# hhcho/sfgwas

Measured on AMD Instinct MI355X. Metric: pca_power_iter_ring_macs_per_s, higher is better.
Workload: dtype u64 ring words, exact integers: int8 digits on the matrix core for the MAC of all five moduli, fp64-held integers in the encode and key-switch kernels

## Files before the change

sfgwas_amd/csrc/fp64mod.hpp:

```cpp
#pragma once

#if defined(__HIPCC__) || defined(__CUDACC__)
#define SFG_HD __host__ __device__ __forceinline__
#else
#define SFG_HD inline
#endif

SFG_HD double mulmod_lazy(double x, double w, double wq, double q) {
    double qh = __builtin_rint(x * wq);
    double h = x * w;
    double l = __builtin_fma(x, w, -h);
    double r = __builtin_fma(-qh, q, h);
    return r + l;
}
SFG_HD double mulmod_lazy_q(double x, double w, double q, double qinv) {
    double h = x * w;
    double qh = __builtin_rint(h * qinv);
    double l = __builtin_fma(x, w, -h);
    double r = __builtin_fma(-qh, q, h);
    return r + l;
}
SFG_HD double canon(double x, double q, double qinv) {
    const double r = __builtin_fma(-__builtin_floor(x * qinv), q, x);
    return r == q ? 0.0 : r;
}
SFG_HD double canon_le(double x, double q, double qinv) {
    return __builtin_fma(-__builtin_floor(x * qinv), q, x);
}
SFG_HD double pred(double x, double q, double qinv) {
    double qh = __builtin_rint(x * qinv);
    return __builtin_fma(-qh, q, x);
}

SFG_HD void fwd_stage1_pair(double v0, double v1, double W, double Wq, double q, double qinv, double &r0, double &r1) {
    const double p = mulmod_lazy(v1, W, Wq, q);
    r0 = canon(v0 + p, q, qinv); r1 = canon(v0 - p, q, qinv);
}
```

sfgwas_amd/csrc/kernels.hpp:

```cpp
#pragma once
#include "common.hpp"
#include "mm_plan.hpp"
#include "assoc_plan.hpp"

constexpr int SFG_MAXPATTERN = 128;
struct ModPattern { int period; int8_t m[SFG_MAXPATTERN]; };
struct RowMap { int rpg; size_t gstride_in, gstride_out; };
struct PanelMap { int G, g, shift0; unsigned packed_mask = 0; int K = 0; };

int launch_ntt_fwd(sfg_ctx *ctx, const u64 *in, u64 *out, size_t nrows, const ModPattern &pat);
int launch_ntt_inv(sfg_ctx *ctx, const u64 *in, u64 *out, size_t nrows, const ModPattern &pat);
int launch_ntt_plain(sfg_ctx *ctx, const double *pc, u64 *out, size_t nplain, int L);
struct MoveJob;
struct PtRide;
int launch_ntt_plain_half(sfg_ctx *ctx, const double *pc, u64 *out_half, size_t nplain, int L, PanelMap pm, const uint32_t *perm = nullptr, const MoveJob *mv = nullptr);
int launch_expand_half(sfg_ctx *ctx, const u64 *half, u64 *full, size_t nrows);
int launch_ntt_fwd_map(sfg_ctx *ctx, const u64 *in, u64 *out, size_t nrows, const ModPattern &pat, const RowMap &rm);
int launch_ntt_inv_map(sfg_ctx *ctx, const u64 *in, u64 *out, size_t nrows, const ModPattern &pat, const RowMap &rm);
int launch_ntt_fwd_staged(sfg_ctx *ctx, const u64 *in, u64 *out, size_t nrows, const ModPattern &pat, bool staged);
struct MacStrides { size_t rot_k, rot_r, pt_k, pt_n, out_n, out_r; bool pt_half = false; bool pt_packed = false; bool pt_digits = false; bool i8 = false; bool i8_big = false; bool pt_digits_big = false;
                    const int8_t *B_small = nullptr, *B_big = nullptr;
                    int pt_layout = 0, pt_L = 0;
                    int B_mode = 0;
                    const int8_t *A_small = nullptr, *A_big = nullptr; };
int launch_mac_i8_small(sfg_ctx *ctx, const double *rotf, size_t rotf_k_stride, size_t rotf_r_stride, int plane0, const u64 *pt, u64 *out, int K, int R, int r0, int Ncols,
                        int l0, int nl, int accumulate, const MacStrides &st);
int launch_mac_i8_big(sfg_ctx *ctx, const double *rotf, size_t rotf_k_stride, size_t rotf_r_stride, int plane0, const u64 *pt, u64 *out, int K, int R, int r0, int Ncols,
                      int l0, int accumulate, const MacStrides &st);
int launch_skew(sfg_ctx *ctx, const int8_t *blk, size_t ld, int r, int c, int transposed, int square, int8_t *D);
struct PcCache { double *slot = nullptr; int mode = 0; const uint32_t *perm = nullptr; };
int launch_encode_rows(sfg_ctx *ctx, const int8_t *D, int shift0, int nshift, int L, u64 *pt, bool half_rows = false, int G = 0, int g = 0, unsigned packed_mask = 0, const PcCache *pcache = nullptr,
                       PtRide *ride = nullptr);
int encode_rows_launches(const sfg_ctx *ctx, int nshift);
int i8_ride_prepare(sfg_ctx *ctx, const u64 *panel, int K, int Ncols, size_t pt_k, size_t pt_n, int layout, int L, int launches, PtRide &ride);
int i8_ride_finish(sfg_ctx *ctx, PtRide &ride);
int i8_ride_tiles(sfg_ctx *ctx, int K, int L, int8_t **Bs, int8_t **Bb);
struct I8Args;
void launch_i8_pack_pt_digits(hipStream_t q, const I8Args &a, unsigned items, bool big);
void launch_move_alone(hipStream_t q, const MoveJob &j);
int launch_share(sfg_ctx *ctx, const u64 *rows, size_t rows_ct_stride, const u64 *xr, size_t x_ct_stride, u64 *h, int nl, int nct);
int launch_add_rows(sfg_ctx *ctx, const u64 *a, size_t a_ct_stride, const u64 *b, size_t b_ct_stride, u64 *out, size_t out_ct_stride, int nl, int nct);
int encrypt_errors_moddown(sfg_ctx *ctx, const int32_t *e0, const int32_t *e1, int nct, int level, u64 *out);
int launch_geno_unpack(sfg_ctx *ctx, const sfg_geno *g, size_t r0, size_t c0, size_t nr, size_t nc, int8_t *out, size_t ld_out);
int launch_rotate_right(sfg_ctx *ctx, const u64 *in, u64 *out, int nct, int level, const int *nrot_host);
int launch_rotate_right_indexed(sfg_ctx *ctx, const u64 *in, int nin, u64 *out, int nct, int level, const int *nrot_host, const int *in_index);
int launch_rotate_right_indexed_f64(sfg_ctx *ctx, const u64 *in, int nin, double *outf, int nct, int level, const int *nrot_host, const int *in_index, int L,
                                    const size_t *out_slot = nullptr);
int launch_rotate_right_sum(sfg_ctx *ctx, const u64 *in, int nin, int nct, int level, const int *nrot_host, const int *in_index, const int *group, int nout,
                            u64 *out, size_t out_stride, int accumulate);
int launch_relinearize(sfg_ctx *ctx, const u64 *tmp, int nct, int level, const u64 *mid, u64 *out);
int launch_ct_add(sfg_ctx *ctx, const u64 *a, const u64 *b, u64 *out, size_t nct, int level);
int mac_dma_planes(sfg_ctx *ctx, int L, std::vector<int> &plane_of, std::vector<int> &is_big);
double mac_big_maxterm(u64 q);
int launch_rot_to_f64(sfg_ctx *ctx, const u64 *rot, size_t nrows, int nl_rot, int L, double *rotf);
int launch_mac_dma(sfg_ctx *ctx, const double *rotf, size_t rows_per_k, const u64 *pt, u64 *out, int K, int R, int Ncols, int L, int accumulate, const MacStrides &st,
                   const double *rotsum = nullptr);
int launch_rot_sum(sfg_ctx *ctx, const double *rotf, size_t rows_per_k, int K, int L, double *rotsum);
int launch_pack_pt(sfg_ctx *ctx, const u64 *in, u64 *out, size_t nrows, size_t words_per_row, int L, unsigned packed_mask);
unsigned mac_dma_packed_mask(sfg_ctx *ctx, int L);
bool mac_use_dma(const sfg_ctx *ctx);
int launch_mac_bc(sfg_ctx *ctx, const double *rotf, size_t rows_per_k, const u64 *pt, u64 *out, int K, int R, int Ncols, int L, int accumulate, const MacStrides &st,
                  const double *rotsum);
int rotcache_build_rows_tab(sfg_ctx *ctx, const u64 *A, int s, int in_level, int max_level, int nbr, int b0, int b1, const std::vector<std::vector<uint8_t>> *tabs, double *cache);
int assoc_build_rotcache(sfg_ctx *ctx, const u64 *A_dev, int s, int in_level, int max_level, size_t nr, const std::vector<size_t> &widths, double **out);
struct I8RotPre { int G = 0, nbr = 0, s = 0, L = 0; std::vector<int8_t *> As, Ab; };
int i8_rotpre_build(sfg_ctx *ctx, const u64 *A_dev, int s, int in_level, int max_level, int nbr, const std::vector<std::vector<uint8_t>> *tabs, size_t budget_bytes, const char *prefix, I8RotPre &pre);
void i8_rotpre_free(I8RotPre &pre);
struct I8RotPreScope { I8RotPre pre; ~I8RotPreScope() { i8_rotpre_free(pre); } };
int matmul_resident_range_i8pre(sfg_ctx *ctx, const I8RotPre &pre, int s, int max_level, const sfg_geno *g, unsigned flags, int blk0, int blk1, uint64_t *out);
int matmul_accumulate_i8pre(sfg_ctx *ctx, const I8RotPre &pre, int s, int max_level, const sfg_geno *g, unsigned flags, int j0, int j1, int accumulate, uint64_t *acc,
                            size_t acc_col_words = 0);
int launch_i8_pack_rot_to(sfg_ctx *ctx, const double *rotf, size_t rotf_k_stride, size_t rotf_r_stride, int plane0, int K, int R, int l0, int nl, bool big, int8_t *A_out);
struct AssocRot { double *f64 = nullptr; I8RotPre pre; };
int assoc_build_rot(sfg_ctx *ctx, const u64 *A_dev, int s, int in_level, int max_level, size_t nr, const std::vector<size_t> &widths, AssocRot &out);
void assoc_free_rot(AssocRot &r);
struct AssocRotScope { AssocRot r; ~AssocRotScope() { assoc_free_rot(r); } };
int assoc_product(sfg_ctx *ctx, const AssocRot &r, const uint64_t *A_dev, int s, int in_level, int max_level, const sfg_geno *g, unsigned flags, int nct, uint64_t *out);
int assoc_batch_tail(sfg_ctx *ctx, const u64 *tmp, const sfg_geno *g, int s, size_t nct, size_t ctw, uint64_t *out_dev, size_t out_ct_capacity, size_t out_shift,
                     double *sum_host, double *sqsum_host);

int launch_bed_decode(sfg_ctx *ctx, hipStream_t st, const uint8_t *dbed, size_t bps, size_t num_sample, size_t num_snp, const int32_t *rmap, const int32_t *cmap,
                      int8_t *out, size_t ld);
int launch_bed_decode_lut(sfg_ctx *ctx, hipStream_t st, const uint8_t *dbed, size_t bps, size_t num_sample, size_t num_snp, const int32_t *rmap, const int32_t *cmap,
                          int8_t *out, size_t ld, unsigned lut);
int upload_filter_map(sfg_ctx *ctx, const uint8_t *filt, size_t n, DevMem &map, size_t *kept);

int assoc_stream_part(sfg_ctx *ctx, int fmt, const char *path, size_t num_sample, size_t num_snp, const uint8_t *row_filter, const uint8_t *col_filter,
                      size_t batch_snps, const uint64_t *A_dev, int s, int in_level, int max_level, unsigned flags,
                      uint64_t *out_dev, size_t out_ct_capacity, size_t *out_ct, double *sum_host, double *sqsum_host,
                      int part, int nparts, std::vector<std::pair<size_t, size_t>> *ranges);
```

sfgwas_amd/csrc/ntt.hip:

```cpp
#include "common.hpp"
#include "kernels.hpp"
#include "i8_move.hpp"
#include "ntt_core.hpp"

template <int IN_MODE>
__global__ void __launch_bounds__(512) k_ntt_fwd(const void *in_, u64 *out_, ModPattern pat, RowMap rm, const double *tw_all, const double2 *pack_all, const ModConst *modc) {
    extern __shared__ double lds[];
    const int N = SFG_N, tid = threadIdx.x;
    const size_t row = blockIdx.x;
    const int m = pat.m[row % pat.period];
    const size_t grp = row / rm.rpg, gi = row % rm.rpg;
    if (m == -2) return;
    if (m < 0) {
        const u64 *src = (const u64 *)in_ + grp * rm.gstride_in + gi * N; u64 *dst = out_ + grp * rm.gstride_out + gi * N;
        if (IN_MODE == 0 && src != dst) for (int a = 0; a < 32; a++) dst[a * 512 + tid] = src[a * 512 + tid];
        return;
    }
    const double *tw = tw_all + (size_t)m * N;
    const double2 *pack = pack_all + (size_t)m * (N / 2);
    const double q = modc[m].q, qinv = modc[m].qinv;
    double v[32];
    if (IN_MODE == 0) {
        const u64 *in = (const u64 *)in_ + grp * rm.gstride_in + gi * N;
#pragma unroll
        for (int a = 0; a < 32; a++) v[a] = u64_to_f64(in[a * 512 + tid]);
    } else {
        const double *pc = (const double *)in_ + (row / pat.period) * (size_t)(N / 2);
#pragma unroll
        for (int a = 0; a < 16; a++) v[a] = pred(pc[a * 512 + tid], q, qinv);
#pragma unroll
        for (int a = 16; a < 32; a++) {
            int x = (a - 16) * 512 + tid;
            v[a] = x == 0 ? 0.0 : -pred(pc[N / 2 - x], q, qinv);
        }
    }
    ntt_fwd_phases(v, lds, tw, pack, q, qinv, tid);
    u64 *out = out_ + grp * rm.gstride_out + gi * N;
    {
        const int b = tid >> 4, c = tid & 15;
#pragma unroll
        for (int a = 0; a < 32; a++) out[a * 512 + tid] = f64_to_u64(canon(lds[a * LDS_ROW + c * 33 + b], q, qinv));
    }
}

__global__ void __launch_bounds__(512) k_ntt_inv(const u64 *in_, u64 *out_, ModPattern pat, RowMap rm, const double *tw_all, const double2 *pack_all, const ModConst *modc) {
    extern __shared__ double lds[];
    const int N = SFG_N, tid = threadIdx.x;
    const size_t row = blockIdx.x;
    const int m = pat.m[row % pat.period];
    if (m < 0) return;
    const size_t grp = row / rm.rpg, gi = row % rm.rpg;
    const double *tw = tw_all + (size_t)m * N;
    const double2 *pack = pack_all + (size_t)m * (N / 2);
    const double q = modc[m].q, qinv = modc[m].qinv;
    const u64 *in = in_ + grp * rm.gstride_in + gi * N;
    double v[32];
    {
        const int b = tid >> 4, c = tid & 15;
#pragma unroll
        for (int a = 0; a < 32; a++) lds[a * LDS_ROW + c * 33 + b] = u64_to_f64(in[a * 512 + tid]);
    }
    __syncthreads();
#pragma unroll
    for (int h = 0; h < 2; h++) {
        const int p = tid + 512 * h, a = p >> 5, b = p & 31;
        double w[16];
#pragma unroll
        for (int c = 0; c < 16; c++) w[c] = lds[a * LDS_ROW + c * 33 + b];
        double tl[16];
        {
            const double2 *pk = pack + (size_t)(p >> 6) * 512 + (p & 63);
#pragma unroll
            for (int i = 0; i < 8; i++) { const double2 e = pk[i * 64]; tl[2 * i] = e.x; tl[2 * i + 1] = e.y; }
        }
        gs_stage<16, 1>(w, q, qinv, [&](int g) { return tl[7 + g]; });
        gs_stage<16, 2>(w, q, qinv, [&](int g) { return tl[3 + g]; });
        gs_stage<16, 4>(w, q, qinv, [&](int g) { return tl[1 + g]; });
        gs_stage<16, 8>(w, q, qinv, [&](int g) { return tl[0 + g]; });
#pragma unroll
        for (int c = 0; c < 16; c++) v[h * 16 + c] = pred(w[c], q, qinv);
    }
    __syncthreads();
#pragma unroll
    for (int h = 0; h < 2; h++) {
        const int p = tid + 512 * h, a = p >> 5, b = p & 31;
#pragma unroll
        for (int c = 0; c < 16; c++) lds[a * LDS_ROW + c * 33 + b] = v[h * 16 + c];
    }
    __syncthreads();
    {
        const int a = tid >> 4, c = tid & 15;
#pragma unroll
        for (int b = 0; b < 32; b++) v[b] = lds[a * LDS_ROW + c * 33 + b];
        gs_stage<32, 1>(v, q, qinv, [&](int g) { return tw[512 + a * 16 + g]; });
        gs_stage<32, 2>(v, q, qinv, [&](int g) { return tw[256 + a * 8 + g]; });
        gs_stage<32, 4>(v, q, qinv, [&](int g) { return tw[128 + a * 4 + g]; });
        gs_stage<32, 8>(v, q, qinv, [&](int g) { return tw[64 + a * 2 + g]; });
        gs_stage<32, 16>(v, q, qinv, [&](int g) { return tw[32 + a + g]; });
        __syncthreads();
#pragma unroll
        for (int b = 0; b < 32; b++) lds[a * LDS_ROW + b * 16 + c] = pred(v[b], q, qinv);
    }
    __syncthreads();
#pragma unroll
    for (int a = 0; a < 32; a++) v[a] = lds[a * LDS_ROW + tid];
    gs_stage<32, 1>(v, q, qinv, [&](int g) { return tw[16 + g]; });
    gs_stage<32, 2>(v, q, qinv, [&](int g) { return tw[8 + g]; });
    gs_stage<32, 4>(v, q, qinv, [&](int g) { return tw[4 + g]; });
    gs_stage<32, 8>(v, q, qinv, [&](int g) { return tw[2 + g]; });
    gs_stage<32, 16>(v, q, qinv, [&](int g) { return tw[1 + g]; });
    const double ninv = modc[m].ninv, ninv_q = modc[m].ninv_q;
    u64 *out = out_ + grp * rm.gstride_out + gi * N;
#pragma unroll
    for (int a = 0; a < 32; a++) {
        double x = mulmod_lazy(pred(v[a], q, qinv), ninv, ninv_q, q);
        out[a * 512 + tid] = f64_to_u64(canon(x, q, qinv));
    }
}

constexpr int H3_ROWA = 264;
constexpr int H3_WREG = 4 * 272;
constexpr int H3_DOUBLES = 16 * H3_ROWA > 4 * H3_WREG ? 16 * H3_ROWA : 4 * H3_WREG;
constexpr int H3_LDS_BYTES = H3_DOUBLES * 8;
struct NoFill {};
template <class First, class Store, class Fill = NoFill, bool WIDE = false>
__device__ __forceinline__ void ntt_half3_body(int hs, First first, Store store, double *lds, const double *tw, const double2 *pack, double q, double qinv, int tid, Fill fill = Fill()) {
    double v[32];
    const int a_b = tid >> 4, c_b = tid & 15;
    double w2[2][16];
    if constexpr (std::is_same<Fill, NoFill>::value) {
#pragma unroll
        for (int h = 0; h < 2; h++)
#pragma unroll
            for (int a = 0; a < 16; a++) w2[h][a] = first(a * 512 + tid + 256 * h);
    } else fill(w2);
#pragma unroll
    for (int h = 0; h < 2; h++) {
        double (&w)[16] = w2[h];
        ct_stage<16, 8>(w, q, qinv, [&](int g) { return tw[2 + hs + g]; });
        ct_stage<16, 4>(w, q, qinv, [&](int g) { return tw[4 + 2 * hs + g]; });
        ct_stage<16, 2>(w, q, qinv, [&](int g) { return tw[8 + 4 * hs + g]; });
        ct_stage<16, 1>(w, q, qinv, [&](int g) { return tw[16 + 8 * hs + g]; });
        if (h) __syncthreads();
#pragma unroll
        for (int a = 0; a < 16; a++) lds[a * H3_ROWA + tid] = w[a];
        __syncthreads();
#pragma unroll
        for (int b = 0; b < 16; b++) v[h * 16 + b] = lds[a_b * H3_ROWA + b * 16 + c_b];
    }
    const int ab = 16 * hs + a_b;
    ct_stage<32, 16>(v, q, qinv, [&](int g) { return tw[32 + ab + g]; });
    ct_stage<32, 8>(v, q, qinv, [&](int g) { return tw[64 + ab * 2 + g]; });
    ct_stage<32, 4>(v, q, qinv, [&](int g) { return tw[128 + ab * 4 + g]; });
    ct_stage<32, 2>(v, q, qinv, [&](int g) { return tw[256 + ab * 8 + g]; });
    ct_stage<32, 1>(v, q, qinv, [&](int g) { return tw[512 + ab * 16 + g]; });
    __syncthreads();
    {
        const int wv = tid >> 6, lane = tid & 63, al = lane >> 4, bk = lane & 15;
        double *img = lds + wv * H3_WREG;
        auto sw = [](int idx) { return (idx >> 8) * 272 + ((idx >> 4) & 15) * 17 + (idx & 15); };
#pragma unroll
        for (int r = 0; r < 2; r++) {
            double wc[16];
            __builtin_amdgcn_fence(__ATOMIC_ACQ_REL, "wavefront");
#pragma unroll
            for (int k = 0; k < 16; k++) img[sw(al * 256 + c_b * 16 + k)] = v[16 * r + k];
            __builtin_amdgcn_fence(__ATOMIC_ACQ_REL, "wavefront");
#pragma unroll
            for (int c = 0; c < 16; c++) wc[c] = img[sw(al * 256 + c * 16 + bk)];
            const int p = a_b * 32 + 16 * r + bk;
            double tl[16];
            {
                const double2 *pk = pack + (size_t)((p >> 6) + 8 * hs) * 512 + (p & 63);
#pragma unroll
                for (int i = 0; i < 8; i++) {
                    const double2 e = pk[i * 64];
                    tl[2 * i] = e.x; tl[2 * i + 1] = e.y;
                }
            }
            ct_stage<16, 8>(wc, q, qinv, [&](int g) { return tl[0 + g]; });
            ct_stage<16, 4>(wc, q, qinv, [&](int g) { return tl[1 + g]; });
            ct_stage<16, 2>(wc, q, qinv, [&](int g) { return tl[3 + g]; });
            ct_stage<16, 1>(wc, q, qinv, [&](int g) { return tl[7 + g]; });
            __builtin_amdgcn_fence(__ATOMIC_ACQ_REL, "wavefront");
#pragma unroll
            for (int c = 0; c < 16; c++) img[sw(al * 256 + c * 16 + bk)] = wc[c];
            __builtin_amdgcn_fence(__ATOMIC_ACQ_REL, "wavefront");
#pragma unroll
            for (int ai = 0; ai < 4; ai++) {
                if constexpr (WIDE) {
                    const int x0 = 4 * lane;
                    const int base = ai * 256 + (lane >> 2);
                    store((4 * wv + ai) * 512 + 256 * r + x0, img[sw(base + (4 * (lane & 3) + 0) * 16)], img[sw(base + (4 * (lane & 3) + 1) * 16)],
                          img[sw(base + (4 * (lane & 3) + 2) * 16)], img[sw(base + (4 * (lane & 3) + 3) * 16)]);
                } else {
#pragma unroll
                    for (int qd = 0; qd < 4; qd++) {
                        const int x = qd * 64 + lane;
                        store((4 * wv + ai) * 512 + 256 * r + x, img[sw(ai * 256 + (x & 15) * 16 + (x >> 4))]);
                    }
                }
            }
        }
    }
}
#define NT_ST(p, v) __builtin_nontemporal_store((unsigned)(v), (p))
template <bool PERM, bool DIG>
__device__ __forceinline__ void ntt_half3_wg(size_t vb, double *lds, const double *pc_all, u64 *out_, size_t nplain, int L, PanelMap pm, const double *tw_all, const double2 *pack_all,
                                             const ModConst *modc, const uint32_t *perm) {
    const int N = SFG_N, n = N / 2, tid = threadIdx.x;
    size_t row; int m;
    if (!plain_block_of(vb, nplain, L, row, m)) return;
    const double *tw = tw_all + (size_t)m * N;
    const double2 *pack = pack_all + (size_t)m * (N / 2);
    const double q = modc[m].q, qinv = modc[m].qinv;
    const double *pc = pc_all + (row / L) * (size_t)n;
    unsigned gal = 1;
    if (PERM) { const uint32_t e = perm[pm.shift0 + (int)(row / L)]; pc = pc_all + (size_t)(e & 0xFFFFu) * n; gal = e >> 16; }
    const double W = tw[1], Wq = W * qinv;
    auto first = [&](int j) { const double lo = pc[j], hi = j == 0 ? 0.0 : pc[n - j]; return lo - mulmod_lazy(hi, W, Wq, q); };
    auto fill = [&](double (&w2)[2][16]) {
        double rA[16], rB[16];
#pragma unroll
        for (int k = 0; k < 16; k++) {
            const int i = tid + 256 * k;
            const double lo = pc[i], hi = i == 0 ? 0.0 : pc[n - i];
            const unsigned qd = (((unsigned)i * gal) & (2u * N - 1u)) >> 13;
            const double ca = (qd == 1u || qd == 2u) ? -lo : lo, cb = qd >= 2u ? -hi : hi;
            rA[k] = ca - mulmod_lazy(cb, W, Wq, q);
            rB[k] = cb - mulmod_lazy(ca, W, Wq, q);
        }
#pragma unroll
        for (int h = 0; h < 2; h++) {
#pragma unroll
            for (int k = 0; k < 16; k++) {
                const unsigned raw = ((unsigned)(tid + 256 * k) * gal) & (2u * N - 1u), qd = raw >> 13;
                const int J = qd == 0u ? (int)raw : qd == 1u ? N - (int)raw : qd == 2u ? (int)raw - N : 2 * N - (int)raw, Jb = n - J;
                if (((J >> 8) & 1) == h && J < n) lds[(J >> 9) * H3_ROWA + (J & 255)] = rA[k];
                if (((Jb >> 8) & 1) == h && Jb < n) lds[(Jb >> 9) * H3_ROWA + (Jb & 255)] = rB[k];
            }
            __syncthreads();
#pragma unroll
            for (int a = 0; a < 16; a++) w2[h][a] = lds[a * H3_ROWA + tid];
            __syncthreads();
        }
        if (tid == 0) {
            const double mid = pc[n / 2];
            const double c = ((((unsigned)(n / 2) * gal) & (2u * N - 1u)) >> 13) >= 2u ? -mid : mid;
            w2[0][8] = c - mulmod_lazy(c, W, Wq, q);
        }
    };
    const size_t plain = row / L; const int shift = pm.shift0 + (int)plain;
    const size_t dst = pm.G ? ((size_t)(shift / SFG_D) * pm.G + pm.g) * SFG_D + (size_t)(shift % SFG_D) : plain;
    u64 *out = out_ + (dst * L + m) * (size_t)n;
    size_t dstride = n, cbm = 0;
    if constexpr (DIG) if (pm.packed_mask & PT_COMPACT) {
        const unsigned lm = (1u << L) - 1u, small = pm.packed_mask & lm;
        const int ns_all = __popc(small), ns_below = __popc(small & ((1u << m) - 1u));
        const size_t planes_all = (size_t)ns_all * 5 + (size_t)(L - ns_all) * 6, planes_below = (size_t)ns_below * 5 + (size_t)(m - ns_below) * 6;
        if (pm.packed_mask & PT_KMAJOR) {
            const size_t K = (size_t)pm.K, col = pm.G ? (size_t)(shift / SFG_D) : plain / K, row = pm.G ? (size_t)pm.g * SFG_D + (size_t)(shift % SFG_D) : plain % K;
            out = reinterpret_cast<u64 *>(reinterpret_cast<uint8_t *>(out_) + ((col * planes_all + planes_below) * 64 * K + row) * 128);
            dstride = 64 * K * 128; cbm = K * 128 - 128;
        } else out = reinterpret_cast<u64 *>(reinterpret_cast<uint8_t *>(out_) + dst * (planes_all * n) + planes_below * n);
    }
    if constexpr (DIG) if (!((pm.packed_mask >> m) & 1u) && (pm.packed_mask & PT_DIGITS_BIG)) {
        uint8_t *o8 = reinterpret_cast<uint8_t *>(out);
        auto dig6 = [&](double x, unsigned &lo, unsigned &hi) {
            const u64 b = (u64)__double_as_longlong(canon(x, q, qinv) + (4503599627370496.0 + 141289400074368.0));
            lo = (unsigned)b ^ 0x80808080u; hi = (unsigned)(b >> 32) ^ 0x8080u;
        };
        auto st6 = [&](int j0, double x0, double x1, double x2, double x3) {
            unsigned l0, l1, l2, l3, h0, h1, h2, h3;
            dig6(x0, l0, h0); dig6(x1, l1, h1); dig6(x2, l2, h2); dig6(x3, l3, h3);
            unsigned o[4]; bytes_tr4(l0, l1, l2, l3, o);
            uint8_t *ob = o8 + j0 + (size_t)(j0 >> 7) * cbm;
#pragma unroll
            for (int d = 0; d < 4; d++) NT_ST(reinterpret_cast<unsigned *>(ob + d * dstride), o[d]);
            unsigned p[4]; bytes_tr4(h0, h1, h2, h3, p);
            NT_ST(reinterpret_cast<unsigned *>(ob + 4 * dstride), p[0]);
            NT_ST(reinterpret_cast<unsigned *>(ob + 5 * dstride), p[1]);
        };
        if constexpr (PERM) ntt_half3_body<decltype(first), decltype(st6), decltype(fill), true>(0, first, st6, lds, tw, pack, q, qinv, tid, fill);
        else ntt_half3_body<decltype(first), decltype(st6), NoFill, true>(0, first, st6, lds, tw, pack, q, qinv, tid);
        return;
    }
    if constexpr (DIG) if ((pm.packed_mask >> m) & 1u) {
        uint8_t *o8 = reinterpret_cast<uint8_t *>(out);
        auto dig = [&](double x, unsigned &lo, unsigned &hi) {
            const u64 b = (u64)__double_as_longlong(canon_le(x, q, qinv) + (4503599627370496.0 + 551911719040.0));
            lo = (unsigned)b ^ 0x80808080u; hi = (unsigned)(b >> 32) ^ 0x80u;
        };
        auto st8 = [&](int j0, double x0, double x1, double x2, double x3) {
            unsigned l0, l1, l2, l3, h0, h1, h2, h3;
            dig(x0, l0, h0); dig(x1, l1, h1); dig(x2, l2, h2); dig(x3, l3, h3);
            unsigned o[4]; bytes_tr4(l0, l1, l2, l3, o);
            uint8_t *ob = o8 + j0 + (size_t)(j0 >> 7) * cbm;
#pragma unroll
            for (int d = 0; d < 4; d++) NT_ST(reinterpret_cast<unsigned *>(ob + d * dstride), o[d]);
            NT_ST(reinterpret_cast<unsigned *>(ob + 4 * dstride), (h0 & 255u) | ((h1 & 255u) << 8) | ((h2 & 255u) << 16) | (h3 << 24));
        };
        if constexpr (PERM) ntt_half3_body<decltype(first), decltype(st8), decltype(fill), true>(0, first, st8, lds, tw, pack, q, qinv, tid, fill);
        else ntt_half3_body<decltype(first), decltype(st8), NoFill, true>(0, first, st8, lds, tw, pack, q, qinv, tid);
        return;
    }
    if constexpr (PERM) {
        if (!DIG && ((pm.packed_mask >> m) & 1u)) ntt_half3_body(0, first, [&](int j, double x) { out[j] = pack_limbs_f64(canon_le(x, q, qinv)); }, lds, tw, pack, q, qinv, tid, fill);
        else ntt_half3_body(0, first, [&](int j, double x) { out[j] = f64_to_u64(canon(x, q, qinv)); }, lds, tw, pack, q, qinv, tid, fill);
    } else {
        (void)fill;
        if (!DIG && ((pm.packed_mask >> m) & 1u)) ntt_half3_body(0, first, [&](int j, double x) { out[j] = pack_limbs_f64(canon_le(x, q, qinv)); }, lds, tw, pack, q, qinv, tid);
        else ntt_half3_body(0, first, [&](int j, double x) { out[j] = f64_to_u64(canon(x, q, qinv)); }, lds, tw, pack, q, qinv, tid);
    }
}
template <bool PERM, bool DIG>
__global__ void __launch_bounds__(256, 4) k_ntt_half3(const double *pc_all, u64 *out_, size_t nplain, int L, PanelMap pm, const double *tw_all, const double2 *pack_all, const ModConst *modc,
                                                      const uint32_t *perm) {
    extern __shared__ double lds[];
    ntt_half3_wg<PERM, DIG>(blockIdx.x, lds, pc_all, out_, nplain, L, pm, tw_all, pack_all, modc, perm);
}
template <bool PERM, int DEPTH, bool NT>
__global__ void __launch_bounds__(256, 4) k_ntt_half3_move(const double *pc_all, u64 *out_, size_t nplain, int L, PanelMap pm, const double *tw_all, const double2 *pack_all, const ModConst *modc,
                                                           const uint32_t *perm, MoveJob job) {
    extern __shared__ double lds[];
    if (blockIdx.x < job.nblocks) { i8_move_block<DEPTH, NT>(job, blockIdx.x, reinterpret_cast<unsigned *>(lds), (int)threadIdx.x); return; }
    ntt_half3_wg<PERM, true>((size_t)blockIdx.x - job.nblocks, lds, pc_all, out_, nplain, L, pm, tw_all, pack_all, modc, perm);
}
template <bool STAGED>
__global__ void __launch_bounds__(256, 4) k_ntt_fwd_split(const u64 *in_, u64 *out_, size_t nrows, ModPattern pat, RowMap rm, const double *tw_all, const double2 *pack_all, const ModConst *modc) {
    extern __shared__ double lds[];
    const int N = SFG_N, n = N / 2, tid = threadIdx.x;
    const size_t b = blockIdx.x, row = (b / 16) * 8 + b % 8; const int hs = (int)((b / 8) & 1);
    if (row >= nrows) return;
    const int m = pat.m[row % pat.period];
    const size_t grp = row / rm.rpg, gi = row % rm.rpg;
    const u64 *in = in_ + grp * rm.gstride_in + gi * N;
    u64 *out = out_ + grp * rm.gstride_out + gi * N + (size_t)hs * n;
    if (m == -2) return;
    if (m < 0) {
        for (int k = 0; k < 32; k++) out[k * 256 + tid] = in[(size_t)hs * n + k * 256 + tid];
        return;
    }
    const double *tw = tw_all + (size_t)m * N;
    const double2 *pack = pack_all + (size_t)m * (N / 2);
    const double q = modc[m].q, qinv = modc[m].qinv;
    const double W = hs ? -tw[1] : tw[1], Wq = W * qinv;
    auto first = [&](int j) { return STAGED ? u64_to_f64(in[(size_t)hs * n + j]) : u64_to_f64(in[j]) + mulmod_lazy(u64_to_f64(in[n + j]), W, Wq, q); };
    ntt_half3_body(hs, first, [&](int j, double x) { out[j] = f64_to_u64(canon(x, q, qinv)); }, lds, tw, pack, q, qinv, tid);
}
__global__ void __launch_bounds__(256) k_expand_half(const u64 *half, u64 *full) {
    const int N = SFG_N, n = N / 2; const size_t row = blockIdx.x / (n / 256);
    const int i = (int)(blockIdx.x % (n / 256)) * 256 + threadIdx.x;
    const u64 v = half[row * n + i];
    full[row * N + i] = v; full[row * N + (N - 1 - i)] = v;
}

int ntt_set_attrs(sfg_ctx *ctx) {
    hipError_t e = hipFuncSetAttribute((const void *)k_ntt_fwd<0>, hipFuncAttributeMaxDynamicSharedMemorySize, LDS_DOUBLES * 8);
    if (e == hipSuccess) e = hipFuncSetAttribute((const void *)k_ntt_fwd<1>, hipFuncAttributeMaxDynamicSharedMemorySize, LDS_DOUBLES * 8);
    if (e == hipSuccess) e = hipFuncSetAttribute((const void *)k_ntt_inv, hipFuncAttributeMaxDynamicSharedMemorySize, LDS_DOUBLES * 8);
    if (e == hipSuccess) e = hipFuncSetAttribute((const void *)k_ntt_half3<false, false>, hipFuncAttributeMaxDynamicSharedMemorySize, H3_LDS_BYTES);
    if (e == hipSuccess) e = hipFuncSetAttribute((const void *)k_ntt_half3<true, false>, hipFuncAttributeMaxDynamicSharedMemorySize, H3_LDS_BYTES);
    if (e == hipSuccess) e = hipFuncSetAttribute((const void *)k_ntt_half3<false, true>, hipFuncAttributeMaxDynamicSharedMemorySize, H3_LDS_BYTES);
    if (e == hipSuccess) e = hipFuncSetAttribute((const void *)k_ntt_half3<true, true>, hipFuncAttributeMaxDynamicSharedMemorySize, H3_LDS_BYTES);
    if (e == hipSuccess) e = hipFuncSetAttribute((const void *)k_ntt_fwd_split<false>, hipFuncAttributeMaxDynamicSharedMemorySize, H3_LDS_BYTES);
    if (e == hipSuccess) e = hipFuncSetAttribute((const void *)k_ntt_fwd_split<true>, hipFuncAttributeMaxDynamicSharedMemorySize, H3_LDS_BYTES);
#define SFG_MV_ATTR(P, D, T) if (e == hipSuccess) e = hipFuncSetAttribute((const void *)k_ntt_half3_move<P, D, T>, hipFuncAttributeMaxDynamicSharedMemorySize, H3_LDS_BYTES)
    SFG_MV_ATTR(false, 1, true); SFG_MV_ATTR(true, 1, true);
#ifdef SFG_AB
    SFG_MV_ATTR(false, 1, false); SFG_MV_ATTR(false, 2, false); SFG_MV_ATTR(false, 2, true); SFG_MV_ATTR(false, 3, false); SFG_MV_ATTR(false, 3, true);
    SFG_MV_ATTR(true, 1, false); SFG_MV_ATTR(true, 2, false); SFG_MV_ATTR(true, 2, true); SFG_MV_ATTR(true, 3, false); SFG_MV_ATTR(true, 3, true);
    if (e == hipSuccess && ab_set_attrs(ctx)) return 1;
#endif
#undef SFG_MV_ATTR
    if (e != hipSuccess) SFG_FAIL(ctx, "cannot raise dynamic LDS limit for the NTT kernels");
    return 0;
}

static RowMap dense_map() { RowMap rm; rm.rpg = 1; rm.gstride_in = SFG_N; rm.gstride_out = SFG_N; return rm; }
int launch_ntt_fwd(sfg_ctx *ctx, const u64 *in, u64 *out, size_t nrows, const ModPattern &pat) { return launch_ntt_fwd_map(ctx, in, out, nrows, pat, dense_map()); }
int launch_ntt_inv(sfg_ctx *ctx, const u64 *in, u64 *out, size_t nrows, const ModPattern &pat) { return launch_ntt_inv_map(ctx, in, out, nrows, pat, dense_map()); }
int launch_ntt_fwd_map(sfg_ctx *ctx, const u64 *in, u64 *out, size_t nrows, const ModPattern &pat, const RowMap &rm) {
    if (!nrows) return 0;
    if (in != out && !ctx->cfg.ntt_fwd_full)
        hipLaunchKernelGGL(k_ntt_fwd_split<false>, dim3((unsigned)((nrows + 7) / 8 * 16)), dim3(256), H3_LDS_BYTES, ctx->stream, in, out, nrows, pat, rm, ctx->tw_fwd, ctx->pack_fwd, ctx->modc);
    else
        hipLaunchKernelGGL(k_ntt_fwd<0>, dim3((unsigned)nrows), dim3(512), LDS_DOUBLES * 8, ctx->stream, (const void *)in, out, pat, rm, ctx->tw_fwd, ctx->pack_fwd, ctx->modc);
    SFG_HIP(ctx, hipGetLastError());
    return 0;
}
int launch_ntt_fwd_staged(sfg_ctx *ctx, const u64 *in, u64 *out, size_t nrows, const ModPattern &pat, bool staged) {
    if (!staged) return launch_ntt_fwd(ctx, in, out, nrows, pat);
    if (!nrows) return 0;
    if (in == out) SFG_FAIL(ctx, "forward NTT: rows staged through stage 1 are transformed out of place");
    hipLaunchKernelGGL(k_ntt_fwd_split<true>, dim3((unsigned)((nrows + 7) / 8 * 16)), dim3(256), H3_LDS_BYTES, ctx->stream, in, out, nrows, pat, dense_map(), ctx->tw_fwd, ctx->pack_fwd, ctx->modc);
    SFG_HIP(ctx, hipGetLastError());
    return 0;
}
int launch_ntt_plain(sfg_ctx *ctx, const double *pc, u64 *out, size_t nplain, int L) {
    if (!nplain) return 0;
    ModPattern pat; pat.period = L; for (int l = 0; l < L; l++) pat.m[l] = (int8_t)l;
    hipLaunchKernelGGL(k_ntt_fwd<1>, dim3((unsigned)(nplain * L)), dim3(512), LDS_DOUBLES * 8, ctx->stream, (const void *)pc, out, pat, dense_map(), ctx->tw_fwd, ctx->pack_fwd, ctx->modc);
    SFG_HIP(ctx, hipGetLastError());
    return 0;
}
template <bool PERM>
static int launch_half3_move(sfg_ctx *ctx, dim3 grid, const double *pc, u64 *out_half, size_t nplain, int L, PanelMap pm, const uint32_t *perm, const MoveJob &j) {
#define SFG_MV(D, T) hipLaunchKernelGGL((k_ntt_half3_move<PERM, D, T>), grid, dim3(256), H3_LDS_BYTES, ctx->stream, pc, out_half, nplain, L, pm, ctx->tw_fwd, ctx->pack_fwd, ctx->modc, perm, j)
    if (j.depth == 1 && j.nt) { SFG_MV(1, true); return 0; }
#ifdef SFG_AB
    if (j.depth == 3) { if (j.nt) SFG_MV(3, true); else SFG_MV(3, false); return 0; }
    if (j.depth == 2) { if (j.nt) SFG_MV(2, true); else SFG_MV(2, false); return 0; }
    if (j.depth == 1) { SFG_MV(1, false); return 0; }
#endif
#undef SFG_MV
    SFG_FAIL(ctx, "plaintext NTT: the product build holds the mover with one unit in flight and streaming accesses only (other forms: make ab)");
}
int launch_ntt_plain_half(sfg_ctx *ctx, const double *pc, u64 *out_half, size_t nplain, int L, PanelMap pm, const uint32_t *perm, const MoveJob *mv) {
    if (!nplain) return 0;
    const dim3 grid((unsigned)((nplain + 7) / 8 * 8 * L));
    const bool dig = pm.packed_mask & PT_DIGITS;
    if (mv && mv->count) {
        if (!dig || mv->nblocks % 8 || !mv->nblocks) SFG_FAIL(ctx, "plaintext NTT: mover workgroups need the digit-plane form and a multiple of 8 of them");
        const dim3 g2(grid.x + mv->nblocks);
        if (perm) SFG_TRY(launch_half3_move<true>(ctx, g2, pc, out_half, nplain, L, pm, perm, *mv));
        else SFG_TRY(launch_half3_move<false>(ctx, g2, pc, out_half, nplain, L, pm, (const uint32_t *)nullptr, *mv));
        SFG_HIP(ctx, hipGetLastError());
        return 0;
    }
    if (perm && dig) hipLaunchKernelGGL((k_ntt_half3<true, true>), grid, dim3(256), H3_LDS_BYTES, ctx->stream, pc, out_half, nplain, L, pm, ctx->tw_fwd, ctx->pack_fwd, ctx->modc, perm);
    else if (perm) hipLaunchKernelGGL((k_ntt_half3<true, false>), grid, dim3(256), H3_LDS_BYTES, ctx->stream, pc, out_half, nplain, L, pm, ctx->tw_fwd, ctx->pack_fwd, ctx->modc, perm);
    else if (dig) hipLaunchKernelGGL((k_ntt_half3<false, true>), grid, dim3(256), H3_LDS_BYTES, ctx->stream, pc, out_half, nplain, L, pm, ctx->tw_fwd, ctx->pack_fwd, ctx->modc, (const uint32_t *)nullptr);
#ifdef SFG_AB
    else if (ctx->cfg.ntt_half_full) ab_launch_ntt_half_full(ctx, pc, out_half, nplain, L, pm);
#endif
    else hipLaunchKernelGGL((k_ntt_half3<false, false>), grid, dim3(256), H3_LDS_BYTES, ctx->stream, pc, out_half, nplain, L, pm, ctx->tw_fwd, ctx->pack_fwd, ctx->modc, (const uint32_t *)nullptr);
    SFG_HIP(ctx, hipGetLastError());
    return 0;
}
int launch_expand_half(sfg_ctx *ctx, const u64 *half, u64 *full, size_t nrows) {
    if (!nrows) return 0;
    hipLaunchKernelGGL(k_expand_half, dim3((unsigned)(nrows * (SFG_N / 2 / 256))), dim3(256), 0, ctx->stream, half, full);
    SFG_HIP(ctx, hipGetLastError());
    return 0;
}
int launch_ntt_inv_map(sfg_ctx *ctx, const u64 *in, u64 *out, size_t nrows, const ModPattern &pat, const RowMap &rm) {
    if (!nrows) return 0;
    hipLaunchKernelGGL(k_ntt_inv, dim3((unsigned)nrows), dim3(512), LDS_DOUBLES * 8, ctx->stream, in, out, pat, rm, ctx->tw_inv, ctx->pack_inv, ctx->modc);
    SFG_HIP(ctx, hipGetLastError());
    return 0;
}

static int pattern_from_host(sfg_ctx *ctx, const int *mod_idx, int nrows, ModPattern &pat) {
    for (int period = 1; period <= 64 && period <= nrows; period++) {
        bool ok = true;
        for (int r = 0; r < nrows && ok; r++) ok = mod_idx[r] == mod_idx[r % period];
        if (ok) { pat.period = period; for (int i = 0; i < period; i++) { if (mod_idx[i] < 0 || mod_idx[i] >= ctx->nmod) SFG_FAIL(ctx, "modulus index out of range"); pat.m[i] = (int8_t)mod_idx[i]; } return 0; }
    }
    SFG_FAIL(ctx, "mod_idx must be periodic with period <= 64");
}

extern "C" int sfg_ntt_rows(sfg_ctx *ctx, uint64_t *rows, int nrows, const int *mod_idx) {
    SFG_HIP(ctx, hipSetDevice(ctx->device));
    ModPattern pat; SFG_TRY(pattern_from_host(ctx, mod_idx, nrows, pat));
    return launch_ntt_fwd(ctx, (const u64 *)rows, (u64 *)rows, nrows, pat);
}
extern "C" int sfg_intt_rows(sfg_ctx *ctx, uint64_t *rows, int nrows, const int *mod_idx) {
    SFG_HIP(ctx, hipSetDevice(ctx->device));
    ModPattern pat; SFG_TRY(pattern_from_host(ctx, mod_idx, nrows, pat));
    return launch_ntt_inv(ctx, (const u64 *)rows, (u64 *)rows, nrows, pat);
}
```

sfgwas_amd/csrc/rotate.hip:

```cpp
#include "common.hpp"
#include "kernels.hpp"
#include "ksw.hpp"


static void fill_ext(const sfg_ctx *ctx, ExtConst &e, const std::vector<int> &src) {
    memset(&e, 0, sizeof e);
    e.a = (int)src.size();
    for (int m = 0; m < e.a; m++) e.src[m] = src[m];
    for (int m = 0; m < e.a; m++) {
        u64 qm = ctx->q[src[m]], h = 1;
        for (int k = 0; k < e.a; k++) if (k != m) h = h_mulmod(h, ctx->q[src[k]] % qm, qm);
        u64 hi = h_invmod(h, qm);
        e.qhat_inv[m] = (double)hi; e.qhat_inv_q[m] = (double)hi / (double)qm;
    }
    for (int t = 0; t < ctx->nmod; t++) {
        u64 qt = ctx->q[t], D = 1 % qt;
        for (int m = 0; m < e.a; m++) {
            u64 ht = 1 % qt;
            for (int k = 0; k < e.a; k++) if (k != m) ht = h_mulmod(ht, ctx->q[src[k]] % qt, qt);
            e.qhat_t[t][m] = (double)ht; e.qhat_t_q[t][m] = (double)ht / (double)qt;
            D = h_mulmod(D, ctx->q[src[m]] % qt, qt);
        }
        e.D_t[t] = (double)D; e.D_t_q[t] = (double)D / (double)qt;
    }
}


int get_ksw(sfg_ctx *ctx, int level, KswConst **dev, KswConst *host) {
    KswConst kc; memset(&kc, 0, sizeof kc);
    kc.level = level; kc.nl = level + 1; kc.np = ctx->np; kc.alpha = ctx->np; kc.nt = kc.nl + kc.np;
    kc.beta = (kc.nl + kc.alpha - 1) / kc.alpha;
    if (kc.alpha > KSW_MAXA || kc.beta > KSW_MAXDIG) SFG_FAIL(ctx, "key-switch shape unsupported (alpha > 4 or beta > 8)");
    if (kc.beta * kc.nt > SFG_MAXPATTERN) SFG_FAIL(ctx, "key-switch shape unsupported (beta * (level + 1 + np) = %d rows exceed the modulus pattern table)", kc.beta * kc.nt);
    for (int t = 0; t < kc.nt; t++) { kc.tmod[t] = t < kc.nl ? t : ctx->nq + (t - kc.nl); kc.digit_of[t] = t < kc.nl ? t / kc.alpha : -1; }
    for (int i = 0; i < kc.beta; i++) {
        std::vector<int> src;
        for (int m = i * kc.alpha; m < (i + 1) * kc.alpha && m < kc.nl; m++) src.push_back(m);
        fill_ext(ctx, kc.dig[i], src);
    }
    std::vector<int> ps; for (int p = 0; p < kc.np; p++) ps.push_back(ctx->nq + p);
    fill_ext(ctx, kc.pq, ps);
    for (int t = 0; t < kc.nl; t++) {
        u64 qt = ctx->q[t], P = 1;
        for (int p = 0; p < kc.np; p++) P = h_mulmod(P, ctx->q[ctx->nq + p] % qt, qt);
        u64 pi = h_invmod(P, qt);
        kc.pinv[t] = (double)pi; kc.pinv_q[t] = (double)pi / (double)qt;
    }
    *host = kc;
    auto it = ctx->ksw_cache.find(level);
    if (it == ctx->ksw_cache.end()) {
        KswConst *d = nullptr;
        SFG_HIP(ctx, hipMalloc(&d, sizeof(KswConst)));
        SFG_HIP(ctx, hipMemcpy(d, &kc, sizeof(KswConst), hipMemcpyHostToDevice));
        ctx->ksw_cache[level] = d; *dev = d;
    } else *dev = (KswConst *)it->second;
    return 0;
}


template <bool PRE1>
__global__ void __launch_bounds__(256) k_ksw_extend(const u64 *c2, u64 *ext, const KswConst *kcp, const ModConst *modc, const double *tw_fwd) {
    const KswConst &kc = *kcp;
    const int N = SFG_N, n = N / 2, x = blockIdx.x * 256 + threadIdx.x, i = blockIdx.y; const size_t b = blockIdx.z;
    const ExtConst &e = kc.dig[i];
    const u64 *c2b = c2 + b * (size_t)kc.nl * N;
    u64 *eb = ext + (b * kc.beta + i) * (size_t)kc.nt * N;
    double xs[2][KSW_MAXA], y[2][KSW_MAXA], v[2] = {0.0, 0.0};
#pragma unroll
    for (int h = 0; h < 2; h++)
#pragma unroll
        for (int m = 0; m < KSW_MAXA; m++) xs[h][m] = m < e.a ? u64_to_f64(c2b[(size_t)e.src[m] * N + h * n + x]) : 0.0;
    if (e.a > 1) { ext_prepare(e, modc, xs[0], y[0], v[0]); ext_prepare(e, modc, xs[1], y[1], v[1]); }
    for (int t = 0; t < kc.nt; t++) {
        const int tg = kc.tmod[t];
        if (kc.digit_of[t] == i) continue;
        const double q = modc[tg].q, qinv = modc[tg].qinv;
        double o0, o1;
        if (e.a == 1) { o0 = canon(xs[0][0], q, qinv); o1 = canon(xs[1][0], q, qinv); }
        else { o0 = ext_target(e, tg, q, qinv, y[0], v[0]); o1 = ext_target(e, tg, q, qinv, y[1], v[1]); }
        if (PRE1) { const double W = tw_fwd[(size_t)tg * N + 1]; fwd_stage1_pair(o0, o1, W, W * qinv, q, qinv, o0, o1); }
        eb[(size_t)t * N + x] = f64_to_u64(o0); eb[(size_t)t * N + n + x] = f64_to_u64(o1);
    }
}

__global__ void __launch_bounds__(256) k_ksw_inner(const u64 *ext, const u64 *ct_in, const u64 *const *keys, const int *inidx, u64 *acc, const KswConst *kcp, const ModConst *modc, int nmod, int nq_out) {
    const KswConst &kc = *kcp;
    const int N = SFG_N, x = 2 * (blockIdx.x * 256 + threadIdx.x), t = (int)blockIdx.y < nq_out ? (int)blockIdx.y : (int)blockIdx.y + (kc.nl - nq_out); const size_t b = blockIdx.z;
    const int tg = kc.tmod[t];
    const double q = modc[tg].q, qinv = modc[tg].qinv;
    const u64 *key = keys[b];
    const size_t bi = (size_t)inidx[b];
    double a0x = 0.0, a0y = 0.0, a1x = 0.0, a1y = 0.0;
    for (int i = 0; i < kc.beta; i++) {
        const ulonglong2 ev = kc.digit_of[t] == i ? *reinterpret_cast<const ulonglong2 *>(ct_in + (bi * 2 * (size_t)kc.nl + kc.nl + t) * N + x)
                                                  : *reinterpret_cast<const ulonglong2 *>(ext + ((bi * kc.beta + i) * (size_t)kc.nt + t) * N + x);
        const ulonglong2 k0 = *reinterpret_cast<const ulonglong2 *>(key + (((size_t)i * 2 + 0) * nmod + tg) * N + x);
        const ulonglong2 k1 = *reinterpret_cast<const ulonglong2 *>(key + (((size_t)i * 2 + 1) * nmod + tg) * N + x);
        const double ex = u64_to_f64(ev.x), ey = u64_to_f64(ev.y);
        a0x += mulmod2(ex, u64_to_f64(k0.x), q, qinv); a0y += mulmod2(ey, u64_to_f64(k0.y), q, qinv);
        a1x += mulmod2(ex, u64_to_f64(k1.x), q, qinv); a1y += mulmod2(ey, u64_to_f64(k1.y), q, qinv);
    }
    *reinterpret_cast<ulonglong2 *>(acc + ((b * 2 + 0) * (size_t)kc.nt + t) * N + x) = make_ulonglong2(f64_to_u64(canon(a0x, q, qinv)), f64_to_u64(canon(a0y, q, qinv)));
    *reinterpret_cast<ulonglong2 *>(acc + ((b * 2 + 1) * (size_t)kc.nt + t) * N + x) = make_ulonglong2(f64_to_u64(canon(a1x, q, qinv)), f64_to_u64(canon(a1y, q, qinv)));
}

template <bool PRE1>
__global__ void __launch_bounds__(256) k_moddown_extend(const u64 *acc, u64 *ext2, const KswConst *kcp, const ModConst *modc, const double *tw_fwd, int nq_out) {
    const KswConst &kc = *kcp;
    const int N = SFG_N, n = N / 2, x = blockIdx.x * 256 + threadIdx.x, p = blockIdx.y; const size_t b = blockIdx.z;
    const ExtConst &e = kc.pq;
    const u64 *ap = acc + ((b * 2 + p) * (size_t)kc.nt + kc.nl) * N;
    double xs[2][KSW_MAXA], y[2][KSW_MAXA], v[2] = {0.0, 0.0};
#pragma unroll
    for (int h = 0; h < 2; h++)
#pragma unroll
        for (int m = 0; m < KSW_MAXA; m++) xs[h][m] = m < e.a ? u64_to_f64(ap[(size_t)m * N + h * n + x]) : 0.0;
    if (e.a > 1) { ext_prepare(e, modc, xs[0], y[0], v[0]); ext_prepare(e, modc, xs[1], y[1], v[1]); }
    for (int t = 0; t < nq_out; t++) {
        const double q = modc[t].q, qinv = modc[t].qinv;
        double o0, o1;
        if (e.a == 1) { o0 = canon(xs[0][0], q, qinv); o1 = canon(xs[1][0], q, qinv); }
        else { o0 = ext_target(e, t, q, qinv, y[0], v[0]); o1 = ext_target(e, t, q, qinv, y[1], v[1]); }
        if (PRE1) { const double W = tw_fwd[(size_t)t * N + 1]; fwd_stage1_pair(o0, o1, W, W * qinv, q, qinv, o0, o1); }
        u64 *row = ext2 + ((b * 2 + p) * (size_t)kc.nl + t) * N;
        row[x] = f64_to_u64(o0); row[n + x] = f64_to_u64(o1);
    }
}

struct F64Form { int on, L, centre; size_t rowf; int plane_of[SFG_MAXMOD], big[SFG_MAXMOD]; };
__device__ __forceinline__ void store_rot_f64(double *row, const F64Form &ff, int t, int x, double v, double q) {
    const int N = SFG_N;
    double *o = row + (size_t)ff.plane_of[t] * N;
    if (ff.big[t]) {
        const double wc = v > __builtin_floor(q * 0.5) ? v - q : v;
        const double hi = __builtin_floor((wc + 4194304.0) * 0x1p-23), lo = wc - hi * 8388608.0;
        o[2 * x] = lo; o[2 * x + 1] = hi;
    } else o[x] = (ff.centre && v > __builtin_floor(q * 0.5)) ? v - q : v;
}
__global__ void __launch_bounds__(256) k_ksw_finish(const u64 *ct_in, const int *inidx, const u64 *acc, const u64 *ext2, const uint16_t *const *index,
                                                   u64 *const *ct_out, const KswConst *kcp, const ModConst *modc, const u64 *add1, F64Form ff) {
    const KswConst &kc = *kcp;
    const int N = SFG_N, x = blockIdx.x * 256 + threadIdx.x, t = blockIdx.y; const size_t b = blockIdx.z;
    if (ff.on && t >= ff.L) return;
    const double q = modc[t].q, qinv = modc[t].qinv, pinv = kc.pinv[t], pinv_q = kc.pinv_q[t];
    const int src = index[b][x];
#pragma unroll
    for (int p = 0; p < 2; p++) {
        const double a = u64_to_f64(acc[((b * 2 + p) * (size_t)kc.nt + t) * N + src]);
        const double e = u64_to_f64(ext2[((b * 2 + p) * (size_t)kc.nl + t) * N + src]);
        double r = mulmod_lazy(a - e, pinv, pinv_q, q);
        if (p == 0) r += u64_to_f64(ct_in[((size_t)inidx[b] * 2 * (size_t)kc.nl + t) * N + src]);
        else if (add1) r += u64_to_f64(add1[((size_t)inidx[b] * (size_t)kc.nl + t) * N + src]);
        const double v = canon(r, q, qinv);
        if (ff.on) store_rot_f64(reinterpret_cast<double *>(ct_out[b]) + (size_t)p * ff.rowf, ff, t, x, v, q);
        else ct_out[b][((size_t)p * kc.nl + t) * N + x] = f64_to_u64(v);
    }
}

struct KswSeg { const u64 *plain; u64 *out; int start, count, accumulate, pad; };
__global__ void __launch_bounds__(256) k_ksw_finish_sum(const u64 *ct_in, const int *inidx, const u64 *acc, const u64 *ext2, const uint16_t *const *index,
                                                       const KswSeg *segs, const int *jobs, const KswConst *kcp, const ModConst *modc) {
    const KswConst &kc = *kcp;
    const int N = SFG_N, x = blockIdx.x * 256 + threadIdx.x, t = blockIdx.y;
    const KswSeg sg = segs[blockIdx.z];
    const double q = modc[t].q, qinv = modc[t].qinv, pinv = kc.pinv[t], pinv_q = kc.pinv_q[t];
    const size_t w0 = (size_t)t * N + x, w1 = ((size_t)kc.nl + t) * N + x;
    double s0 = 0.0, s1 = 0.0;
    if (sg.accumulate) { s0 = u64_to_f64(sg.out[w0]); s1 = u64_to_f64(sg.out[w1]); }
    if (sg.plain) { s0 += u64_to_f64(sg.plain[w0]); s1 += u64_to_f64(sg.plain[w1]); }
    for (int k = 0; k < sg.count; k++) {
        const size_t b = (size_t)jobs[sg.start + k];
        const int src = index[b][x];
        const double a0 = u64_to_f64(acc[((b * 2 + 0) * (size_t)kc.nt + t) * N + src]), e0 = u64_to_f64(ext2[((b * 2 + 0) * (size_t)kc.nl + t) * N + src]);
        const double a1 = u64_to_f64(acc[((b * 2 + 1) * (size_t)kc.nt + t) * N + src]), e1 = u64_to_f64(ext2[((b * 2 + 1) * (size_t)kc.nl + t) * N + src]);
        const double c0 = u64_to_f64(ct_in[((size_t)inidx[b] * 2 * (size_t)kc.nl + t) * N + src]);
        s0 += canon(mulmod_lazy(a0 - e0, pinv, pinv_q, q) + c0, q, qinv);
        s1 += canon(mulmod_lazy(a1 - e1, pinv, pinv_q, q), q, qinv);
        if ((k & 7) == 7) { s0 = pred(s0, q, qinv); s1 = pred(s1, q, qinv); }
    }
    sg.out[w0] = f64_to_u64(canon(s0, q, qinv)); sg.out[w1] = f64_to_u64(canon(s1, q, qinv));
}

__global__ void __launch_bounds__(256) k_ct_add(const u64 *a, const u64 *b, u64 *out, int nl, const ModConst *modc, size_t total_rows) {
    const int N = SFG_N; const size_t row = blockIdx.x / (N / 256); const int m = (int)(row % nl);
    const u64 q = modc[m].qi;
    const size_t off = row * N + (blockIdx.x % (N / 256)) * 256 + threadIdx.x;
    u64 v = a[off] + b[off]; out[off] = v >= q ? v - q : v;
}

struct KswSum { int nout; std::vector<int> group; std::vector<const u64 *> plain; u64 *out; size_t out_stride; int accumulate; };
static int launch_keyswitch_jobs(sfg_ctx *ctx, const u64 *in, int nin, int level, const std::vector<int> &job_in, const std::vector<const u64 *> &keyp,
                                 const std::vector<const uint16_t *> &idxp, const std::vector<u64 *> &outp, const u64 *add1, const F64Form *ffp = nullptr,
                                 const KswSum *sum = nullptr) {
    const int N = SFG_N, nl = level + 1;
    F64Form ff; memset(&ff, 0, sizeof ff); if (ffp) ff = *ffp;
    KswConst *kcd; KswConst kc;
    SFG_TRY(get_ksw(ctx, level, &kcd, &kc));
    const size_t ctw = (size_t)2 * nl * N;
    const int nr = (int)job_in.size(), nout = sum ? sum->nout : 0;
    if (sum && (ff.on || add1 || (int)sum->group.size() != nr || (int)sum->plain.size() != nout)) SFG_FAIL(ctx, "key switch: internal: malformed sum groups");
    if (!nr && !nout) return 0;
    const int nq_out = ff.on ? ff.L : nl;
    const bool pre1 = !ctx->cfg.ntt_fwd_full;
    const size_t in_rows = (size_t)nl + (size_t)kc.beta * kc.nt, job_rows = 2 * (size_t)kc.nt + 2 * (size_t)nl;
    const size_t budget = ctx->cfg.ksw_budget;
    int in_grp = (int)(budget / (in_rows * N * 8)); if (in_grp < 1) in_grp = 1; if (in_grp > nin) in_grp = nin;
    int chunk = (int)(budget / (job_rows * N * 8)); if (chunk < 1) chunk = 1; if (chunk > nr) chunk = nr;
    const size_t ptr_bytes = (size_t)nr * (3 * sizeof(void *) + 2 * sizeof(int)) + (size_t)nout * sizeof(KswSeg) + 256;
    const size_t ext_rows = (size_t)in_grp * kc.beta * kc.nt, ext2_rows = (size_t)chunk * 2 * nl;
    SFG_TRY(sfg_ws_reserve(ctx, (in_rows * in_grp + job_rows * chunk + ext_rows + ext2_rows) * N * 8 + ptr_bytes));
    u64 *c2 = (u64 *)ctx->ws, *ext = c2 + (size_t)in_grp * nl * N;
    u64 *acc = ext + ext_rows * N, *ext2 = acc + (size_t)chunk * 2 * kc.nt * N;
    u64 *extT = ext2 + ext2_rows * N, *ext2T = extT + ext_rows * N;
    const u64 **keys_all = (const u64 **)(ext2T + ext2_rows * N);
    const uint16_t **idx_all = (const uint16_t **)(keys_all + nr);
    u64 **out_all = (u64 **)(idx_all + nr);
    KswSeg *segs_d = (KswSeg *)(out_all + nr);
    int *inidx_all = (int *)(segs_d + nout);
    int *segjobs_d = inidx_all + nr;
    std::vector<char> seen(nout, 0);
    std::vector<KswSeg> segs; std::vector<int> segjobs;
    auto finish_sum = [&](const std::vector<int> &jobs, size_t c0, int nb, const u64 *bin, const int *inidx_d, const uint16_t **idx_d) -> int {
        std::vector<int> cnt(nout, 0), at(nout, 0);
        for (int k = 0; k < nb; k++) cnt[sum->group[jobs[c0 + k]]]++;
        segs.clear(); segjobs.assign(nb, 0);
        for (int i = 0, start = 0; i < nout; i++) {
            if (nb ? !cnt[i] : seen[i]) continue;
            KswSeg sg; sg.plain = seen[i] ? nullptr : sum->plain[i]; sg.out = sum->out + (size_t)i * sum->out_stride;
            sg.start = start; sg.count = cnt[i]; sg.accumulate = (sum->accumulate || seen[i]) ? 1 : 0; sg.pad = 0;
            at[i] = start; start += cnt[i]; seen[i] = 1; segs.push_back(sg);
        }
        for (int k = 0; k < nb; k++) segjobs[at[sum->group[jobs[c0 + k]]]++] = k;
        if (segs.empty()) return 0;
        SFG_TRY(sfg_upload_small(ctx, segs_d, segs.data(), segs.size() * sizeof(KswSeg)));
        SFG_TRY(sfg_upload_small(ctx, segjobs_d, segjobs.data(), (size_t)nb * sizeof(int)));
        hipLaunchKernelGGL(k_ksw_finish_sum, dim3(N / 256, nl, (unsigned)segs.size()), dim3(256), 0, ctx->stream, bin, inidx_d, acc, ext2T, idx_d, segs_d, segjobs_d, kcd, ctx->modc);
        SFG_HIP(ctx, hipGetLastError());
        return 0;
    };
    ModPattern pq; pq.period = nl; for (int m = 0; m < nl; m++) pq.m[m] = m < nq_out ? (int8_t)m : (int8_t)-2;
    ModPattern pin; pin.period = nl; for (int m = 0; m < nl; m++) pin.m[m] = (int8_t)m;
    ModPattern pext; pext.period = kc.beta * kc.nt;
    for (int i = 0; i < kc.beta; i++) for (int t = 0; t < kc.nt; t++)
        pext.m[i * kc.nt + t] = (kc.digit_of[t] == i || (t >= nq_out && t < nl)) ? (int8_t)-2 : (int8_t)kc.tmod[t];
    ModPattern pp; pp.period = kc.np; for (int p = 0; p < kc.np; p++) pp.m[p] = (int8_t)(ctx->nq + p);
    for (int i0 = 0; i0 < nin; i0 += in_grp) {
        const int ni = nin - i0 < in_grp ? nin - i0 : in_grp;
        std::vector<int> jobs;
        for (int k = 0; k < nr; k++) if (job_in[k] >= i0 && job_in[k] < i0 + ni) jobs.push_back(k);
        if (jobs.empty()) continue;
        const u64 *bin = in + (size_t)i0 * ctw;
        RowMap rm1; rm1.rpg = nl; rm1.gstride_in = ctw; rm1.gstride_out = (size_t)nl * N;
        SFG_TRY(launch_ntt_inv_map(ctx, bin + (size_t)nl * N, c2, (size_t)ni * nl, pin, rm1));
        if (pre1) hipLaunchKernelGGL(k_ksw_extend<true>, dim3(N / 512, kc.beta, ni), dim3(256), 0, ctx->stream, c2, ext, kcd, ctx->modc, ctx->tw_fwd);
        else hipLaunchKernelGGL(k_ksw_extend<false>, dim3(N / 512, kc.beta, ni), dim3(256), 0, ctx->stream, c2, ext, kcd, ctx->modc, ctx->tw_fwd);
        SFG_HIP(ctx, hipGetLastError());
        SFG_TRY(launch_ntt_fwd_staged(ctx, ext, extT, (size_t)ni * kc.beta * kc.nt, pext, pre1));
        {
            const size_t nj = jobs.size();
            std::vector<const u64 *> kp(nj); std::vector<const uint16_t *> ip(nj); std::vector<u64 *> op(nj); std::vector<int> ii(nj);
            for (size_t k = 0; k < nj; k++) { int jb = jobs[k]; kp[k] = keyp[jb]; ip[k] = idxp[jb]; op[k] = sum ? nullptr : outp[jb]; ii[k] = job_in[jb] - i0; }
            SFG_TRY(sfg_upload_small(ctx, keys_all, kp.data(), nj * sizeof(void *)));
            SFG_TRY(sfg_upload_small(ctx, idx_all, ip.data(), nj * sizeof(void *)));
            if (!sum) SFG_TRY(sfg_upload_small(ctx, out_all, op.data(), nj * sizeof(void *)));
            SFG_TRY(sfg_upload_small(ctx, inidx_all, ii.data(), nj * sizeof(int)));
        }
        for (size_t c0 = 0; c0 < jobs.size(); c0 += chunk) {
            const int nb = (int)(jobs.size() - c0 < (size_t)chunk ? jobs.size() - c0 : (size_t)chunk);
            const u64 **keys_d = keys_all + c0; const uint16_t **idx_d = idx_all + c0; u64 **out_d = out_all + c0; int *inidx_d = inidx_all + c0;
            hipLaunchKernelGGL(k_ksw_inner, dim3(N / 512, nq_out + kc.np, nb), dim3(256), 0, ctx->stream, extT, bin, keys_d, inidx_d, acc, kcd, ctx->modc, ctx->nmod, nq_out);
            SFG_HIP(ctx, hipGetLastError());
            RowMap rm4; rm4.rpg = kc.np; rm4.gstride_in = (size_t)kc.nt * N; rm4.gstride_out = (size_t)kc.nt * N;
            SFG_TRY(launch_ntt_inv_map(ctx, acc + (size_t)nl * N, acc + (size_t)nl * N, (size_t)nb * 2 * kc.np, pp, rm4));
            if (pre1) hipLaunchKernelGGL(k_moddown_extend<true>, dim3(N / 512, 2, nb), dim3(256), 0, ctx->stream, acc, ext2, kcd, ctx->modc, ctx->tw_fwd, nq_out);
            else hipLaunchKernelGGL(k_moddown_extend<false>, dim3(N / 512, 2, nb), dim3(256), 0, ctx->stream, acc, ext2, kcd, ctx->modc, ctx->tw_fwd, nq_out);
            SFG_HIP(ctx, hipGetLastError());
            SFG_TRY(launch_ntt_fwd_staged(ctx, ext2, ext2T, (size_t)nb * 2 * nl, pq, pre1));
            if (sum) { SFG_TRY(finish_sum(jobs, c0, nb, bin, inidx_d, idx_d)); continue; }
            hipLaunchKernelGGL(k_ksw_finish, dim3(N / 256, nq_out, nb), dim3(256), 0, ctx->stream, bin, inidx_d, acc, ext2T, idx_d, out_d, kcd, ctx->modc,
                               add1 ? add1 + (size_t)i0 * nl * N : nullptr, ff);
            SFG_HIP(ctx, hipGetLastError());
        }
    }
    if (sum) SFG_TRY(finish_sum(std::vector<int>(), 0, 0, in, inidx_all, idx_all));
    return 0;
}
int launch_rotate_right_indexed(sfg_ctx *ctx, const u64 *in, int nin, u64 *out, int nct, int level, const int *nrot_host, const int *in_index) {
    const int N = SFG_N, nl = level + 1;
    if (level < 0 || level >= ctx->nq) SFG_FAIL(ctx, "rotate: level out of range");
    const size_t ctw = (size_t)2 * nl * N;
    std::vector<int> job_in; std::vector<const u64 *> keyp; std::vector<const uint16_t *> idxp; std::vector<u64 *> outp;
    for (int j = 0; j < nct; j++) {
        int nrot = nrot_host[j] % SFG_SLOTS; if (nrot < 0) nrot += SFG_SLOTS;
        const int src = in_index ? in_index[j] : j;
        if (src < 0 || src >= nin) SFG_FAIL(ctx, "rotate: input index out of range");
        if (nrot == 0) {
            int run = 1;
            while (j + run < nct && (nrot_host[j + run] % SFG_SLOTS) == 0 && (in_index ? in_index[j + run] : j + run) == src + run && src + run < nin) run++;
            SFG_HIP(ctx, hipMemcpyAsync(out + j * ctw, in + (size_t)src * ctw, (size_t)run * ctw * 8, hipMemcpyDeviceToDevice, ctx->stream));
            j += run - 1;
            continue;
        }
        u64 g = sfg_galois_for_rotation(ctx, SFG_SLOTS - nrot);
        auto it = ctx->rotkeys().find(g);
        if (it == ctx->rotkeys().end()) SFG_FAIL(ctx, "rotate: no rotation key loaded for right-rotation by %d (galois element %llu)", nrot, g);
        job_in.push_back(src); keyp.push_back(it->second.key_dev); idxp.push_back(it->second.index_dev); outp.push_back(out + j * ctw);
    }
    return launch_keyswitch_jobs(ctx, in, nin, level, job_in, keyp, idxp, outp, nullptr);
}
int launch_rotate_right_sum(sfg_ctx *ctx, const u64 *in, int nin, int nct, int level, const int *nrot_host, const int *in_index, const int *group, int nout,
                            u64 *out, size_t out_stride, int accumulate) {
    const int N = SFG_N, nl = level + 1;
    if (level < 0 || level >= ctx->nq) SFG_FAIL(ctx, "rotate: level out of range");
    const size_t ctw = (size_t)2 * nl * N;
    KswSum sum; sum.nout = nout; sum.plain.assign(nout, nullptr); sum.out = out; sum.out_stride = out_stride; sum.accumulate = accumulate;
    std::vector<int> job_in; std::vector<const u64 *> keyp; std::vector<const uint16_t *> idxp;
    for (int j = 0; j < nct; j++) {
        int nrot = nrot_host[j] % SFG_SLOTS; if (nrot < 0) nrot += SFG_SLOTS;
        const int src = in_index ? in_index[j] : j;
        if (src < 0 || src >= nin) SFG_FAIL(ctx, "rotate: input index out of range");
        if (group[j] < 0 || group[j] >= nout) SFG_FAIL(ctx, "rotate: sum group out of range");
        if (nrot == 0) {
            if (sum.plain[group[j]]) SFG_FAIL(ctx, "rotate: more than one unrotated member in a sum group");
            sum.plain[group[j]] = in + (size_t)src * ctw;
            continue;
        }
        u64 g = sfg_galois_for_rotation(ctx, SFG_SLOTS - nrot);
        auto it = ctx->rotkeys().find(g);
        if (it == ctx->rotkeys().end()) SFG_FAIL(ctx, "rotate: no rotation key loaded for right-rotation by %d (galois element %llu)", nrot, g);
        job_in.push_back(src); keyp.push_back(it->second.key_dev); idxp.push_back(it->second.index_dev); sum.group.push_back(group[j]);
    }
    return launch_keyswitch_jobs(ctx, in, nin, level, job_in, keyp, idxp, std::vector<u64 *>(), nullptr, nullptr, &sum);
}
int launch_rotate_right_indexed_f64(sfg_ctx *ctx, const u64 *in, int nin, double *outf, int nct, int level, const int *nrot_host, const int *in_index, int L,
                                    const size_t *out_slot) {
    const int N = SFG_N, nl = level + 1;
    ctx->i8_gen++;
    if (level < 0 || level >= ctx->nq || L > nl) SFG_FAIL(ctx, "rotate: level out of range");
    const size_t ctw = (size_t)2 * nl * N;
    std::vector<int> plane_of, is_big; const int nplanes = mac_dma_planes(ctx, L, plane_of, is_big);
    if (nplanes < 0) return 1;
    F64Form ff; memset(&ff, 0, sizeof ff);
    ff.on = 1; ff.L = L; ff.centre = mac_dma_packed_mask(ctx, L) != 0; ff.rowf = (size_t)nplanes * N;
    for (int l = 0; l < L; l++) { ff.plane_of[l] = plane_of[l]; ff.big[l] = is_big[l]; }
    std::vector<int> job_in; std::vector<const u64 *> keyp; std::vector<const uint16_t *> idxp; std::vector<u64 *> outp;
    for (int j = 0; j < nct; j++) {
        int nrot = nrot_host[j] % SFG_SLOTS; if (nrot < 0) nrot += SFG_SLOTS;
        const int src = in_index ? in_index[j] : j;
        if (src < 0 || src >= nin) SFG_FAIL(ctx, "rotate: input index out of range");
        double *dst = outf + (out_slot ? out_slot[j] : (size_t)j) * 2 * ff.rowf;
        if (nrot == 0) {
            int run = 1;
            while (!out_slot && j + run < nct && (nrot_host[j + run] % SFG_SLOTS) == 0 && (in_index ? in_index[j + run] : j + run) == src + run && src + run < nin) run++;
            SFG_TRY(launch_rot_to_f64(ctx, in + (size_t)src * ctw, (size_t)2 * run, nl, L, dst));
            j += run - 1;
            continue;
        }
        u64 g = sfg_galois_for_rotation(ctx, SFG_SLOTS - nrot);
        auto it = ctx->rotkeys().find(g);
        if (it == ctx->rotkeys().end()) SFG_FAIL(ctx, "rotate: no rotation key loaded for right-rotation by %d (galois element %llu)", nrot, g);
        job_in.push_back(src); keyp.push_back(it->second.key_dev); idxp.push_back(it->second.index_dev); outp.push_back(reinterpret_cast<u64 *>(dst));
    }
    return launch_keyswitch_jobs(ctx, in, nin, level, job_in, keyp, idxp, outp, nullptr, &ff);
}
int launch_relinearize(sfg_ctx *ctx, const u64 *tmp, int nct, int level, const u64 *mid, u64 *out) {
    auto it = ctx->rotkeys().find(1);
    if (it == ctx->rotkeys().end()) SFG_FAIL(ctx, "relinearize: no relinearisation key loaded");
    const size_t ctw = (size_t)2 * (level + 1) * SFG_N;
    std::vector<int> job_in(nct); std::vector<const u64 *> keyp(nct, it->second.key_dev); std::vector<const uint16_t *> idxp(nct, it->second.index_dev); std::vector<u64 *> outp(nct);
    for (int j = 0; j < nct; j++) { job_in[j] = j; outp[j] = out + (size_t)j * ctw; }
    return launch_keyswitch_jobs(ctx, tmp, nct, level, job_in, keyp, idxp, outp, mid);
}
int launch_rotate_right(sfg_ctx *ctx, const u64 *in, u64 *out, int nct, int level, const int *nrot_host) {
    return launch_rotate_right_indexed(ctx, in, nct, out, nct, level, nrot_host, nullptr);
}

extern "C" int sfg_rotate_right_dev(sfg_ctx *ctx, const uint64_t *in, uint64_t *out, int nct, int level, const int *nrot_host) {
    SFG_HIP(ctx, hipSetDevice(ctx->device));
    if (in == out) SFG_FAIL(ctx, "rotate: in and out must not alias");
    PhaseTimer t(ctx, "rotate");
    int rc = launch_rotate_right(ctx, (const u64 *)in, (u64 *)out, nct, level, nrot_host);
    t.stop(1);
    return rc;
}

extern "C" int sfg_ct_galois_dev(sfg_ctx *ctx, const uint64_t *in, uint64_t *out, int nct, int level, uint64_t galois_el) {
    SFG_HIP(ctx, hipSetDevice(ctx->device));
    if (in == out) SFG_FAIL(ctx, "galois: in and out must not alias");
    if (level < 0 || level >= ctx->nq) SFG_FAIL(ctx, "galois: level out of range");
    auto it = ctx->rotkeys().find(galois_el);
    if (it == ctx->rotkeys().end() || galois_el == 1) SFG_FAIL(ctx, "galois: no switching key loaded for galois element %llu", (unsigned long long)galois_el);
    const size_t ctw = (size_t)2 * (level + 1) * SFG_N;
    std::vector<int> job_in(nct); std::vector<const u64 *> keyp(nct, it->second.key_dev); std::vector<const uint16_t *> idxp(nct, it->second.index_dev); std::vector<u64 *> outp(nct);
    for (int j = 0; j < nct; j++) { job_in[j] = j; outp[j] = (u64 *)out + (size_t)j * ctw; }
    PhaseTimer t(ctx, "rotate");
    int rc = launch_keyswitch_jobs(ctx, (const u64 *)in, nct, level, job_in, keyp, idxp, outp, nullptr);
    t.stop(1);
    return rc;
}

int launch_ct_add(sfg_ctx *ctx, const u64 *a, const u64 *b, u64 *out, size_t nct, int level) {
    const int nl = level + 1; const size_t rows = nct * 2 * nl;
    if (!rows) return 0;
    hipLaunchKernelGGL(k_ct_add, dim3((unsigned)(rows * (SFG_N / 256))), dim3(256), 0, ctx->stream, a, b, out, nl, ctx->modc, rows);
    SFG_HIP(ctx, hipGetLastError());
    return 0;
}
extern "C" int sfg_ct_add_dev(sfg_ctx *ctx, const uint64_t *a, const uint64_t *b, uint64_t *out, int nct, int level) {
    SFG_HIP(ctx, hipSetDevice(ctx->device));
    if (level < 0 || level >= ctx->nq) SFG_FAIL(ctx, "evaluator op: level %d out of range", level);
    if (nct < 0) SFG_FAIL(ctx, "evaluator op: negative ciphertext count");
    return launch_ct_add(ctx, (const u64 *)a, (const u64 *)b, (u64 *)out, (size_t)nct, level);
}
```

Baseline: 6342 billion.

## Restructure key-switch: split inverse NTT, tile jobs sharing keys, fuse q-part inner product into finish

Adds a split inverse NTT kernel that leaves the last butterfly stage undone, folding it into the extend and moddown kernels that follow. The key-switch inner product now groups consecutive jobs that share a key and index table into tiles of up to three, so each key load serves several ciphertexts. The inner kernel now covers only the special primes, while the q-modulus inner product is recomputed inside the finish kernels. This is meant to cut key memory traffic, launch work and accumulator size, at the cost of more complex kernels and more register pressure.

After: 6481 billion, median of 6. 1.02x the previous value.

```diff
diff --git a/sfgwas_amd/csrc/fp64mod.hpp b/sfgwas_amd/csrc/fp64mod.hpp
--- a/sfgwas_amd/csrc/fp64mod.hpp
+++ b/sfgwas_amd/csrc/fp64mod.hpp
@@ -36,3 +36,6 @@
     const double p = mulmod_lazy(v1, W, Wq, q);
     r0 = canon(v0 + p, q, qinv); r1 = canon(v0 - p, q, qinv);
 }
+SFG_HD void inv_last_pair(double U, double V, double ninv, double ninv_q, double wn, double wn_q, double q, double qinv, double &r0, double &r1) {
+    r0 = canon(mulmod_lazy(U + V, ninv, ninv_q, q), q, qinv); r1 = canon(mulmod_lazy(U - V, wn, wn_q, q), q, qinv);
+}
diff --git a/sfgwas_amd/csrc/kernels.hpp b/sfgwas_amd/csrc/kernels.hpp
--- a/sfgwas_amd/csrc/kernels.hpp
+++ b/sfgwas_amd/csrc/kernels.hpp
@@ -18,6 +18,7 @@
 int launch_ntt_fwd_map(sfg_ctx *ctx, const u64 *in, u64 *out, size_t nrows, const ModPattern &pat, const RowMap &rm);
 int launch_ntt_inv_map(sfg_ctx *ctx, const u64 *in, u64 *out, size_t nrows, const ModPattern &pat, const RowMap &rm);
 int launch_ntt_fwd_staged(sfg_ctx *ctx, const u64 *in, u64 *out, size_t nrows, const ModPattern &pat, bool staged);
+int launch_ntt_inv_split(sfg_ctx *ctx, const u64 *in, u64 *out, size_t nrows, const ModPattern &pat, const RowMap &rm);
 struct MacStrides { size_t rot_k, rot_r, pt_k, pt_n, out_n, out_r; bool pt_half = false; bool pt_packed = false; bool pt_digits = false; bool i8 = false; bool i8_big = false; bool pt_digits_big = false;
                     const int8_t *B_small = nullptr, *B_big = nullptr;
                     int pt_layout = 0, pt_L = 0;
diff --git a/sfgwas_amd/csrc/ksw_plan.hpp b/sfgwas_amd/csrc/ksw_plan.hpp
--- /dev/null
+++ b/sfgwas_amd/csrc/ksw_plan.hpp
@@ -0,0 +1,30 @@
+#pragma once
+#include <cstddef>
+#include <vector>
+
+struct KswTile { int start, count; };
+
+template <class K, class I>
+inline void ksw_job_tiles(const K *key, const I *tab, int nb, int T, std::vector<KswTile> &tiles) {
+    tiles.clear();
+    if (T < 1) T = 1;
+    for (int k = 0; k < nb;) {
+        int n = 1;
+        while (k + n < nb && n < T && key[k + n] == key[k] && tab[k + n] == tab[k]) n++;
+        tiles.push_back(KswTile{k, n});
+        k += n;
+    }
+}
+
+struct KswSegPlan { int out, start, count, first; };
+inline void ksw_plan_segments(const int *group, int nb, int nout, std::vector<char> &seen, std::vector<KswSegPlan> &segs, std::vector<int> &segjobs) {
+    std::vector<int> cnt((size_t)nout, 0), at((size_t)nout, 0);
+    for (int k = 0; k < nb; k++) cnt[(size_t)group[k]]++;
+    segs.clear(); segjobs.assign((size_t)nb, 0);
+    for (int i = 0, start = 0; i < nout; i++) {
+        if (nb ? !cnt[(size_t)i] : (bool)seen[(size_t)i]) continue;
+        segs.push_back(KswSegPlan{i, start, cnt[(size_t)i], seen[(size_t)i] ? 0 : 1});
+        at[(size_t)i] = start; start += cnt[(size_t)i]; seen[(size_t)i] = 1;
+    }
+    for (int k = 0; k < nb; k++) segjobs[(size_t)at[(size_t)group[k]]++] = k;
+}
diff --git a/sfgwas_amd/csrc/ntt.hip b/sfgwas_amd/csrc/ntt.hip
--- a/sfgwas_amd/csrc/ntt.hip
+++ b/sfgwas_amd/csrc/ntt.hip
@@ -348,6 +348,82 @@
     auto first = [&](int j) { return STAGED ? u64_to_f64(in[(size_t)hs * n + j]) : u64_to_f64(in[j]) + mulmod_lazy(u64_to_f64(in[n + j]), W, Wq, q); };
     ntt_half3_body(hs, first, [&](int j, double x) { out[j] = f64_to_u64(canon(x, q, qinv)); }, lds, tw, pack, q, qinv, tid);
 }
+__global__ void __launch_bounds__(256, 4) k_ntt_inv_split(const u64 *in_, u64 *out_, size_t nrows, ModPattern pat, RowMap rm, const double *tw_all, const double2 *pack_all, const ModConst *modc) {
+    extern __shared__ double lds[];
+    const int N = SFG_N, n = N / 2, tid = threadIdx.x;
+    const size_t blk = blockIdx.x, row = (blk / 16) * 8 + blk % 8; const int hs = (int)((blk / 8) & 1);
+    if (row >= nrows) return;
+    const int m = pat.m[row % pat.period];
+    if (m < 0) return;
+    const size_t grp = row / rm.rpg, gi = row % rm.rpg;
+    const u64 *in = in_ + grp * rm.gstride_in + gi * N + (size_t)hs * n;
+    u64 *out = out_ + grp * rm.gstride_out + gi * N + (size_t)hs * n;
+    const double *tw = tw_all + (size_t)m * N;
+    const double2 *pack = pack_all + (size_t)m * (N / 2);
+    const double q = modc[m].q, qinv = modc[m].qinv;
+    const int a_b = tid >> 4, c_b = tid & 15;
+    double v[32];
+    {
+        const int wv = tid >> 6, lane = tid & 63, al = lane >> 4, bk = lane & 15;
+        double *img = lds + wv * H3_WREG;
+        auto sw = [](int idx) { return (idx >> 8) * 272 + ((idx >> 4) & 15) * 17 + (idx & 15); };
+#pragma unroll
+        for (int r = 0; r < 2; r++) {
+            double wc[16];
+            __builtin_amdgcn_fence(__ATOMIC_ACQ_REL, "wavefront");
+#pragma unroll
+            for (int ai = 0; ai < 4; ai++)
+#pragma unroll
+                for (int qd = 0; qd < 4; qd++) {
+                    const int x = qd * 64 + lane;
+                    img[sw(ai * 256 + (x & 15) * 16 + (x >> 4))] = u64_to_f64(in[(4 * wv + ai) * 512 + 256 * r + x]);
+                }
+            __builtin_amdgcn_fence(__ATOMIC_ACQ_REL, "wavefront");
+#pragma unroll
+            for (int c = 0; c < 16; c++) wc[c] = img[sw(al * 256 + c * 16 + bk)];
+            const int p = a_b * 32 + 16 * r + bk;
+            double tl[16];
+            {
+                const double2 *pk = pack + (size_t)((p >> 6) + 8 * hs) * 512 + (p & 63);
+#pragma unroll
+                for (int i = 0; i < 8; i++) { const double2 e = pk[i * 64]; tl[2 * i] = e.x; tl[2 * i + 1] = e.y; }
+            }
+            gs_stage<16, 1>(wc, q, qinv, [&](int g) { return tl[7 + g]; });
+            gs_stage<16, 2>(wc, q, qinv, [&](int g) { return tl[3 + g]; });
+            gs_stage<16, 4>(wc, q, qinv, [&](int g) { return tl[1 + g]; });
+            gs_stage<16, 8>(wc, q, qinv, [&](int g) { return tl[0 + g]; });
+            __builtin_amdgcn_fence(__ATOMIC_ACQ_REL, "wavefront");
+#pragma unroll
+            for (int c = 0; c < 16; c++) img[sw(al * 256 + c * 16 + bk)] = pred(wc[c], q, qinv);
+            __builtin_amdgcn_fence(__ATOMIC_ACQ_REL, "wavefront");
+#pragma unroll
+            for (int k = 0; k < 16; k++) v[16 * r + k] = img[sw(al * 256 + c_b * 16 + k)];
+        }
+    }
+    const int ab = 16 * hs + a_b;
+    gs_stage<32, 1>(v, q, qinv, [&](int g) { return tw[512 + ab * 16 + g]; });
+    gs_stage<32, 2>(v, q, qinv, [&](int g) { return tw[256 + ab * 8 + g]; });
+    gs_stage<32, 4>(v, q, qinv, [&](int g) { return tw[128 + ab * 4 + g]; });
+    gs_stage<32, 8>(v, q, qinv, [&](int g) { return tw[64 + ab * 2 + g]; });
+    gs_stage<32, 16>(v, q, qinv, [&](int g) { return tw[32 + ab + g]; });
+    __syncthreads();
+#pragma unroll
+    for (int h = 0; h < 2; h++) {
+        double w[16];
+        if (h) __syncthreads();
+#pragma unroll
+        for (int b = 0; b < 16; b++) lds[a_b * H3_ROWA + b * 16 + c_b] = pred(v[h * 16 + b], q, qinv);
+        __syncthreads();
+#pragma unroll
+        for (int a = 0; a < 16; a++) w[a] = lds[a * H3_ROWA + tid];
+        gs_stage<16, 1>(w, q, qinv, [&](int g) { return tw[16 + 8 * hs + g]; });
+        gs_stage<16, 2>(w, q, qinv, [&](int g) { return tw[8 + 4 * hs + g]; });
+        gs_stage<16, 4>(w, q, qinv, [&](int g) { return tw[4 + 2 * hs + g]; });
+        gs_stage<16, 8>(w, q, qinv, [&](int g) { return tw[2 + hs + g]; });
+#pragma unroll
+        for (int a = 0; a < 16; a++) out[a * 512 + tid + 256 * h] = f64_to_u64(canon(w[a], q, qinv));
+    }
+}
 __global__ void __launch_bounds__(256) k_expand_half(const u64 *half, u64 *full) {
     const int N = SFG_N, n = N / 2; const size_t row = blockIdx.x / (n / 256);
     const int i = (int)(blockIdx.x % (n / 256)) * 256 + threadIdx.x;
@@ -365,6 +441,7 @@
     if (e == hipSuccess) e = hipFuncSetAttribute((const void *)k_ntt_half3<true, true>, hipFuncAttributeMaxDynamicSharedMemorySize, H3_LDS_BYTES);
     if (e == hipSuccess) e = hipFuncSetAttribute((const void *)k_ntt_fwd_split<false>, hipFuncAttributeMaxDynamicSharedMemorySize, H3_LDS_BYTES);
     if (e == hipSuccess) e = hipFuncSetAttribute((const void *)k_ntt_fwd_split<true>, hipFuncAttributeMaxDynamicSharedMemorySize, H3_LDS_BYTES);
+    if (e == hipSuccess) e = hipFuncSetAttribute((const void *)k_ntt_inv_split, hipFuncAttributeMaxDynamicSharedMemorySize, H3_LDS_BYTES);
 #define SFG_MV_ATTR(P, D, T) if (e == hipSuccess) e = hipFuncSetAttribute((const void *)k_ntt_half3_move<P, D, T>, hipFuncAttributeMaxDynamicSharedMemorySize, H3_LDS_BYTES)
     SFG_MV_ATTR(false, 1, true); SFG_MV_ATTR(true, 1, true);
 #ifdef SFG_AB
@@ -450,6 +527,12 @@
     SFG_HIP(ctx, hipGetLastError());
     return 0;
 }
+int launch_ntt_inv_split(sfg_ctx *ctx, const u64 *in, u64 *out, size_t nrows, const ModPattern &pat, const RowMap &rm) {
+    if (!nrows) return 0;
+    hipLaunchKernelGGL(k_ntt_inv_split, dim3((unsigned)((nrows + 7) / 8 * 16)), dim3(256), H3_LDS_BYTES, ctx->stream, in, out, nrows, pat, rm, ctx->tw_inv, ctx->pack_inv, ctx->modc);
+    SFG_HIP(ctx, hipGetLastError());
+    return 0;
+}
 
 static int pattern_from_host(sfg_ctx *ctx, const int *mod_idx, int nrows, ModPattern &pat) {
     for (int period = 1; period <= 64 && period <= nrows; period++) {
diff --git a/sfgwas_amd/csrc/rotate.hip b/sfgwas_amd/csrc/rotate.hip
--- a/sfgwas_amd/csrc/rotate.hip
+++ b/sfgwas_amd/csrc/rotate.hip
@@ -1,6 +1,14 @@
 #include "common.hpp"
 #include "kernels.hpp"
 #include "ksw.hpp"
+#include "ksw_plan.hpp"
+
+#ifndef KSW_T
+#define KSW_T 3
+#endif
+#ifndef KSW_INV_SPLIT
+#define KSW_INV_SPLIT true
+#endif
 
 
 static void fill_ext(const sfg_ctx *ctx, ExtConst &e, const std::vector<int> &src) {
@@ -58,8 +66,12 @@
 }
 
 
-template <bool PRE1>
-__global__ void __launch_bounds__(256) k_ksw_extend(const u64 *c2, u64 *ext, const KswConst *kcp, const ModConst *modc, const double *tw_fwd) {
+__device__ __forceinline__ void inv_last_of(const ModConst &mc, double w, double &u, double &v) {
+    const double wn = canon(mulmod_lazy(w, mc.ninv, mc.ninv_q, mc.q), mc.q, mc.qinv);
+    inv_last_pair(u, v, mc.ninv, mc.ninv_q, wn, wn * mc.qinv, mc.q, mc.qinv, u, v);
+}
+template <bool PRE1, bool POST1>
+__global__ void __launch_bounds__(256) k_ksw_extend(const u64 *c2, u64 *ext, const KswConst *kcp, const ModConst *modc, const double *tw_fwd, const double *tw_inv) {
     const KswConst &kc = *kcp;
     const int N = SFG_N, n = N / 2, x = blockIdx.x * 256 + threadIdx.x, i = blockIdx.y; const size_t b = blockIdx.z;
     const ExtConst &e = kc.dig[i];
@@ -70,6 +82,10 @@
     for (int h = 0; h < 2; h++)
 #pragma unroll
         for (int m = 0; m < KSW_MAXA; m++) xs[h][m] = m < e.a ? u64_to_f64(c2b[(size_t)e.src[m] * N + h * n + x]) : 0.0;
+    if (POST1) {
+#pragma unroll
+        for (int m = 0; m < KSW_MAXA; m++) if (m < e.a) inv_last_of(modc[e.src[m]], tw_inv[(size_t)e.src[m] * N + 1], xs[0][m], xs[1][m]);
+    }
     if (e.a > 1) { ext_prepare(e, modc, xs[0], y[0], v[0]); ext_prepare(e, modc, xs[1], y[1], v[1]); }
     for (int t = 0; t < kc.nt; t++) {
         const int tg = kc.tmod[t];
@@ -83,38 +99,58 @@
     }
 }
 
-__global__ void __launch_bounds__(256) k_ksw_inner(const u64 *ext, const u64 *ct_in, const u64 *const *keys, const int *inidx, u64 *acc, const KswConst *kcp, const ModConst *modc, int nmod, int nq_out) {
+template <int T>
+__global__ void __launch_bounds__(256) k_ksw_inner_p(const u64 *ext, const u64 *const *keys, const int *inidx, const KswTile *tiles, u64 *acc, const KswConst *kcp,
+                                                    const ModConst *modc, int nmod) {
     const KswConst &kc = *kcp;
-    const int N = SFG_N, x = 2 * (blockIdx.x * 256 + threadIdx.x), t = (int)blockIdx.y < nq_out ? (int)blockIdx.y : (int)blockIdx.y + (kc.nl - nq_out); const size_t b = blockIdx.z;
+    const int N = SFG_N, x = 2 * (blockIdx.x * 256 + threadIdx.x), m = blockIdx.y, t = kc.nl + m;
+    const KswTile tl = tiles[blockIdx.z];
     const int tg = kc.tmod[t];
     const double q = modc[tg].q, qinv = modc[tg].qinv;
-    const u64 *key = keys[b];
-    const size_t bi = (size_t)inidx[b];
-    double a0x = 0.0, a0y = 0.0, a1x = 0.0, a1y = 0.0;
+    const u64 *key = keys[tl.start];
+    const u64 *eb[T];
+#pragma unroll
+    for (int j = 0; j < T; j++) eb[j] = ext + ((size_t)inidx[tl.start + (j < tl.count ? j : 0)] * kc.beta * (size_t)kc.nt + t) * N + x;
+    double a[T][4];
+#pragma unroll
+    for (int j = 0; j < T; j++) a[j][0] = a[j][1] = a[j][2] = a[j][3] = 0.0;
     for (int i = 0; i < kc.beta; i++) {
-        const ulonglong2 ev = kc.digit_of[t] == i ? *reinterpret_cast<const ulonglong2 *>(ct_in + (bi * 2 * (size_t)kc.nl + kc.nl + t) * N + x)
-                                                  : *reinterpret_cast<const ulonglong2 *>(ext + ((bi * kc.beta + i) * (size_t)kc.nt + t) * N + x);
         const ulonglong2 k0 = *reinterpret_cast<const ulonglong2 *>(key + (((size_t)i * 2 + 0) * nmod + tg) * N + x);
         const ulonglong2 k1 = *reinterpret_cast<const ulonglong2 *>(key + (((size_t)i * 2 + 1) * nmod + tg) * N + x);
-        const double ex = u64_to_f64(ev.x), ey = u64_to_f64(ev.y);
-        a0x += mulmod2(ex, u64_to_f64(k0.x), q, qinv); a0y += mulmod2(ey, u64_to_f64(k0.y), q, qinv);
-        a1x += mulmod2(ex, u64_to_f64(k1.x), q, qinv); a1y += mulmod2(ey, u64_to_f64(k1.y), q, qinv);
-    }
-    *reinterpret_cast<ulonglong2 *>(acc + ((b * 2 + 0) * (size_t)kc.nt + t) * N + x) = make_ulonglong2(f64_to_u64(canon(a0x, q, qinv)), f64_to_u64(canon(a0y, q, qinv)));
-    *reinterpret_cast<ulonglong2 *>(acc + ((b * 2 + 1) * (size_t)kc.nt + t) * N + x) = make_ulonglong2(f64_to_u64(canon(a1x, q, qinv)), f64_to_u64(canon(a1y, q, qinv)));
-}
-
-template <bool PRE1>
-__global__ void __launch_bounds__(256) k_moddown_extend(const u64 *acc, u64 *ext2, const KswConst *kcp, const ModConst *modc, const double *tw_fwd, int nq_out) {
+        const double k0x = u64_to_f64(k0.x), k0y = u64_to_f64(k0.y), k1x = u64_to_f64(k1.x), k1y = u64_to_f64(k1.y);
+#pragma unroll
+        for (int j = 0; j < T; j++) {
+            const ulonglong2 ev = *reinterpret_cast<const ulonglong2 *>(eb[j] + (size_t)i * kc.nt * N);
+            const double ex = u64_to_f64(ev.x), ey = u64_to_f64(ev.y);
+            a[j][0] += mulmod2(ex, k0x, q, qinv); a[j][1] += mulmod2(ey, k0y, q, qinv);
+            a[j][2] += mulmod2(ex, k1x, q, qinv); a[j][3] += mulmod2(ey, k1y, q, qinv);
+        }
+    }
+#pragma unroll
+    for (int j = 0; j < T; j++) {
+        if (j < tl.count) {
+            u64 *o = acc + ((size_t)(tl.start + j) * 2 * kc.np + m) * N + x;
+            *reinterpret_cast<ulonglong2 *>(o) = make_ulonglong2(f64_to_u64(canon(a[j][0], q, qinv)), f64_to_u64(canon(a[j][1], q, qinv)));
+            *reinterpret_cast<ulonglong2 *>(o + (size_t)kc.np * N) = make_ulonglong2(f64_to_u64(canon(a[j][2], q, qinv)), f64_to_u64(canon(a[j][3], q, qinv)));
+        }
+    }
+}
+
+template <bool PRE1, bool POST1>
+__global__ void __launch_bounds__(256) k_moddown_extend(const u64 *acc, u64 *ext2, const KswConst *kcp, const ModConst *modc, const double *tw_fwd, const double *tw_inv, int nq_out) {
     const KswConst &kc = *kcp;
     const int N = SFG_N, n = N / 2, x = blockIdx.x * 256 + threadIdx.x, p = blockIdx.y; const size_t b = blockIdx.z;
     const ExtConst &e = kc.pq;
-    const u64 *ap = acc + ((b * 2 + p) * (size_t)kc.nt + kc.nl) * N;
+    const u64 *ap = acc + (b * 2 + p) * (size_t)kc.np * N;
     double xs[2][KSW_MAXA], y[2][KSW_MAXA], v[2] = {0.0, 0.0};
 #pragma unroll
     for (int h = 0; h < 2; h++)
 #pragma unroll
         for (int m = 0; m < KSW_MAXA; m++) xs[h][m] = m < e.a ? u64_to_f64(ap[(size_t)m * N + h * n + x]) : 0.0;
+    if (POST1) {
+#pragma unroll
+        for (int m = 0; m < KSW_MAXA; m++) if (m < e.a) inv_last_of(modc[e.src[m]], tw_inv[(size_t)e.src[m] * N + 1], xs[0][m], xs[1][m]);
+    }
     if (e.a > 1) { ext_prepare(e, modc, xs[0], y[0], v[0]); ext_prepare(e, modc, xs[1], y[1], v[1]); }
     for (int t = 0; t < nq_out; t++) {
         const double q = modc[t].q, qinv = modc[t].qinv;
@@ -137,29 +173,57 @@
         o[2 * x] = lo; o[2 * x + 1] = hi;
     } else o[x] = (ff.centre && v > __builtin_floor(q * 0.5)) ? v - q : v;
 }
-__global__ void __launch_bounds__(256) k_ksw_finish(const u64 *ct_in, const int *inidx, const u64 *acc, const u64 *ext2, const uint16_t *const *index,
-                                                   u64 *const *ct_out, const KswConst *kcp, const ModConst *modc, const u64 *add1, F64Form ff) {
+template <int T>
+__device__ __forceinline__ void ksw_inner_q(const u64 *ext, const u64 *ct_in, const u64 *key, const KswConst &kc, int nmod, int t, int src, const size_t (&bi)[T],
+                                           double q, double qinv, double (&a)[T][2]) {
+    const int N = SFG_N;
+#pragma unroll
+    for (int j = 0; j < T; j++) a[j][0] = a[j][1] = 0.0;
+    for (int i = 0; i < kc.beta; i++) {
+        const double k0 = u64_to_f64(key[(((size_t)i * 2 + 0) * nmod + t) * N + src]), k1 = u64_to_f64(key[(((size_t)i * 2 + 1) * nmod + t) * N + src]);
+        const bool own = kc.digit_of[t] == i;
+#pragma unroll
+        for (int j = 0; j < T; j++) {
+            const double e = u64_to_f64(own ? ct_in[(bi[j] * 2 * (size_t)kc.nl + kc.nl + t) * N + src] : ext[((bi[j] * kc.beta + i) * (size_t)kc.nt + t) * N + src]);
+            a[j][0] += mulmod2(e, k0, q, qinv); a[j][1] += mulmod2(e, k1, q, qinv);
+        }
+    }
+}
+template <int T>
+__global__ void __launch_bounds__(256) k_ksw_finish(const u64 *ext, const u64 *ct_in, const u64 *const *keys, const int *inidx, const u64 *ext2, const uint16_t *const *index,
+                                                   u64 *const *ct_out, const KswTile *tiles, const KswConst *kcp, const ModConst *modc, int nmod, const u64 *add1, F64Form ff) {
     const KswConst &kc = *kcp;
-    const int N = SFG_N, x = blockIdx.x * 256 + threadIdx.x, t = blockIdx.y; const size_t b = blockIdx.z;
+    const int N = SFG_N, x = blockIdx.x * 256 + threadIdx.x, t = blockIdx.y;
     if (ff.on && t >= ff.L) return;
+    const KswTile tl = tiles[blockIdx.z];
     const double q = modc[t].q, qinv = modc[t].qinv, pinv = kc.pinv[t], pinv_q = kc.pinv_q[t];
-    const int src = index[b][x];
-#pragma unroll
-    for (int p = 0; p < 2; p++) {
-        const double a = u64_to_f64(acc[((b * 2 + p) * (size_t)kc.nt + t) * N + src]);
-        const double e = u64_to_f64(ext2[((b * 2 + p) * (size_t)kc.nl + t) * N + src]);
-        double r = mulmod_lazy(a - e, pinv, pinv_q, q);
-        if (p == 0) r += u64_to_f64(ct_in[((size_t)inidx[b] * 2 * (size_t)kc.nl + t) * N + src]);
-        else if (add1) r += u64_to_f64(add1[((size_t)inidx[b] * (size_t)kc.nl + t) * N + src]);
-        const double v = canon(r, q, qinv);
-        if (ff.on) store_rot_f64(reinterpret_cast<double *>(ct_out[b]) + (size_t)p * ff.rowf, ff, t, x, v, q);
-        else ct_out[b][((size_t)p * kc.nl + t) * N + x] = f64_to_u64(v);
+    const int src = index[tl.start][x];
+    size_t bi[T];
+#pragma unroll
+    for (int j = 0; j < T; j++) bi[j] = (size_t)inidx[tl.start + (j < tl.count ? j : 0)];
+    double a[T][2];
+    ksw_inner_q<T>(ext, ct_in, keys[tl.start], kc, nmod, t, src, bi, q, qinv, a);
+#pragma unroll
+    for (int j = 0; j < T; j++) {
+        if (j < tl.count) {
+            const size_t b = (size_t)(tl.start + j);
+#pragma unroll
+            for (int p = 0; p < 2; p++) {
+                const double e = u64_to_f64(ext2[((b * 2 + p) * (size_t)kc.nl + t) * N + src]);
+                double r = mulmod_lazy(pred(a[j][p], q, qinv) - e, pinv, pinv_q, q);
+                if (p == 0) r += u64_to_f64(ct_in[(bi[j] * 2 * (size_t)kc.nl + t) * N + src]);
+                else if (add1) r += u64_to_f64(add1[(bi[j] * (size_t)kc.nl + t) * N + src]);
+                const double v = canon(r, q, qinv);
+                if (ff.on) store_rot_f64(reinterpret_cast<double *>(ct_out[b]) + (size_t)p * ff.rowf, ff, t, x, v, q);
+                else ct_out[b][((size_t)p * kc.nl + t) * N + x] = f64_to_u64(v);
+            }
+        }
     }
 }
 
 struct KswSeg { const u64 *plain; u64 *out; int start, count, accumulate, pad; };
-__global__ void __launch_bounds__(256) k_ksw_finish_sum(const u64 *ct_in, const int *inidx, const u64 *acc, const u64 *ext2, const uint16_t *const *index,
-                                                       const KswSeg *segs, const int *jobs, const KswConst *kcp, const ModConst *modc) {
+__global__ void __launch_bounds__(256) k_ksw_finish_sum(const u64 *ext, const u64 *ct_in, const u64 *const *keys, const int *inidx, const u64 *ext2, const uint16_t *const *index,
+                                                       const KswSeg *segs, const int *jobs, const KswConst *kcp, const ModConst *modc, int nmod) {
     const KswConst &kc = *kcp;
     const int N = SFG_N, x = blockIdx.x * 256 + threadIdx.x, t = blockIdx.y;
     const KswSeg sg = segs[blockIdx.z];
@@ -170,12 +234,14 @@
     if (sg.plain) { s0 += u64_to_f64(sg.plain[w0]); s1 += u64_to_f64(sg.plain[w1]); }
     for (int k = 0; k < sg.count; k++) {
         const size_t b = (size_t)jobs[sg.start + k];
+        const size_t bi[1] = {(size_t)inidx[b]};
         const int src = index[b][x];
-        const double a0 = u64_to_f64(acc[((b * 2 + 0) * (size_t)kc.nt + t) * N + src]), e0 = u64_to_f64(ext2[((b * 2 + 0) * (size_t)kc.nl + t) * N + src]);
-        const double a1 = u64_to_f64(acc[((b * 2 + 1) * (size_t)kc.nt + t) * N + src]), e1 = u64_to_f64(ext2[((b * 2 + 1) * (size_t)kc.nl + t) * N + src]);
-        const double c0 = u64_to_f64(ct_in[((size_t)inidx[b] * 2 * (size_t)kc.nl + t) * N + src]);
-        s0 += canon(mulmod_lazy(a0 - e0, pinv, pinv_q, q) + c0, q, qinv);
-        s1 += canon(mulmod_lazy(a1 - e1, pinv, pinv_q, q), q, qinv);
+        double a[1][2];
+        ksw_inner_q<1>(ext, ct_in, keys[b], kc, nmod, t, src, bi, q, qinv, a);
+        const double e0 = u64_to_f64(ext2[((b * 2 + 0) * (size_t)kc.nl + t) * N + src]), e1 = u64_to_f64(ext2[((b * 2 + 1) * (size_t)kc.nl + t) * N + src]);
+        const double c0 = u64_to_f64(ct_in[(bi[0] * 2 * (size_t)kc.nl + t) * N + src]);
+        s0 += canon(mulmod_lazy(pred(a[0][0], q, qinv) - e0, pinv, pinv_q, q) + c0, q, qinv);
+        s1 += canon(mulmod_lazy(pred(a[0][1], q, qinv) - e1, pinv, pinv_q, q), q, qinv);
         if ((k & 7) == 7) { s0 = pred(s0, q, qinv); s1 = pred(s1, q, qinv); }
     }
     sg.out[w0] = f64_to_u64(canon(s0, q, qinv)); sg.out[w1] = f64_to_u64(canon(s1, q, qinv));
@@ -206,11 +272,11 @@
     const size_t budget = ctx->cfg.ksw_budget;
     int in_grp = (int)(budget / (in_rows * N * 8)); if (in_grp < 1) in_grp = 1; if (in_grp > nin) in_grp = nin;
     int chunk = (int)(budget / (job_rows * N * 8)); if (chunk < 1) chunk = 1; if (chunk > nr) chunk = nr;
-    const size_t ptr_bytes = (size_t)nr * (3 * sizeof(void *) + 2 * sizeof(int)) + (size_t)nout * sizeof(KswSeg) + 256;
-    const size_t ext_rows = (size_t)in_grp * kc.beta * kc.nt, ext2_rows = (size_t)chunk * 2 * nl;
-    SFG_TRY(sfg_ws_reserve(ctx, (in_rows * in_grp + job_rows * chunk + ext_rows + ext2_rows) * N * 8 + ptr_bytes));
+    const size_t ptr_bytes = (size_t)nr * (3 * sizeof(void *) + 2 * sizeof(int) + sizeof(KswTile)) + (size_t)nout * sizeof(KswSeg) + 256;
+    const size_t ext_rows = (size_t)in_grp * kc.beta * kc.nt, ext2_rows = (size_t)chunk * 2 * nl, acc_rows = (size_t)chunk * 2 * kc.np;
+    SFG_TRY(sfg_ws_reserve(ctx, (in_rows * in_grp + acc_rows + 2 * ext2_rows + ext_rows) * N * 8 + ptr_bytes));
     u64 *c2 = (u64 *)ctx->ws, *ext = c2 + (size_t)in_grp * nl * N;
-    u64 *acc = ext + ext_rows * N, *ext2 = acc + (size_t)chunk * 2 * kc.nt * N;
+    u64 *acc = ext + ext_rows * N, *ext2 = acc + acc_rows * N;
     u64 *extT = ext2 + ext2_rows * N, *ext2T = extT + ext_rows * N;
     const u64 **keys_all = (const u64 **)(ext2T + ext2_rows * N);
     const uint16_t **idx_all = (const uint16_t **)(keys_all + nr);
@@ -218,23 +284,24 @@
     KswSeg *segs_d = (KswSeg *)(out_all + nr);
     int *inidx_all = (int *)(segs_d + nout);
     int *segjobs_d = inidx_all + nr;
+    KswTile *tiles_all = (KswTile *)(segjobs_d + nr);
     std::vector<char> seen(nout, 0);
-    std::vector<KswSeg> segs; std::vector<int> segjobs;
-    auto finish_sum = [&](const std::vector<int> &jobs, size_t c0, int nb, const u64 *bin, const int *inidx_d, const uint16_t **idx_d) -> int {
-        std::vector<int> cnt(nout, 0), at(nout, 0);
-        for (int k = 0; k < nb; k++) cnt[sum->group[jobs[c0 + k]]]++;
-        segs.clear(); segjobs.assign(nb, 0);
-        for (int i = 0, start = 0; i < nout; i++) {
-            if (nb ? !cnt[i] : seen[i]) continue;
-            KswSeg sg; sg.plain = seen[i] ? nullptr : sum->plain[i]; sg.out = sum->out + (size_t)i * sum->out_stride;
-            sg.start = start; sg.count = cnt[i]; sg.accumulate = (sum->accumulate || seen[i]) ? 1 : 0; sg.pad = 0;
-            at[i] = start; start += cnt[i]; seen[i] = 1; segs.push_back(sg);
-        }
-        for (int k = 0; k < nb; k++) segjobs[at[sum->group[jobs[c0 + k]]]++] = k;
-        if (segs.empty()) return 0;
+    std::vector<KswSegPlan> plan; std::vector<KswSeg> segs; std::vector<int> segjobs, grp;
+    auto finish_sum = [&](const std::vector<int> &jobs, size_t c0, int nb, const u64 *bin, const u64 **keys_d, const int *inidx_d, const uint16_t **idx_d) -> int {
+        grp.resize(nb);
+        for (int k = 0; k < nb; k++) grp[k] = sum->group[jobs[c0 + k]];
+        ksw_plan_segments(grp.data(), nb, nout, seen, plan, segjobs);
+        if (plan.empty()) return 0;
+        segs.clear();
+        for (const KswSegPlan &sp : plan) {
+            KswSeg sg; sg.plain = sp.first ? sum->plain[sp.out] : nullptr; sg.out = sum->out + (size_t)sp.out * sum->out_stride;
+            sg.start = sp.start; sg.count = sp.count; sg.accumulate = (sum->accumulate || !sp.first) ? 1 : 0; sg.pad = 0;
+            segs.push_back(sg);
+        }
         SFG_TRY(sfg_upload_small(ctx, segs_d, segs.data(), segs.size() * sizeof(KswSeg)));
         SFG_TRY(sfg_upload_small(ctx, segjobs_d, segjobs.data(), (size_t)nb * sizeof(int)));
-        hipLaunchKernelGGL(k_ksw_finish_sum, dim3(N / 256, nl, (unsigned)segs.size()), dim3(256), 0, ctx->stream, bin, inidx_d, acc, ext2T, idx_d, segs_d, segjobs_d, kcd, ctx->modc);
+        hipLaunchKernelGGL(k_ksw_finish_sum, dim3(N / 256, nl, (unsigned)segs.size()), dim3(256), 0, ctx->stream, extT, bin, keys_d, inidx_d, ext2T, idx_d,
+                           segs_d, segjobs_d, kcd, ctx->modc, ctx->nmod);
         SFG_HIP(ctx, hipGetLastError());
         return 0;
     };
@@ -244,6 +311,7 @@
     for (int i = 0; i < kc.beta; i++) for (int t = 0; t < kc.nt; t++)
         pext.m[i * kc.nt + t] = (kc.digit_of[t] == i || (t >= nq_out && t < nl)) ? (int8_t)-2 : (int8_t)kc.tmod[t];
     ModPattern pp; pp.period = kc.np; for (int p = 0; p < kc.np; p++) pp.m[p] = (int8_t)(ctx->nq + p);
+    RowMap rm_dense; rm_dense.rpg = 1; rm_dense.gstride_in = N; rm_dense.gstride_out = N;
     for (int i0 = 0; i0 < nin; i0 += in_grp) {
         const int ni = nin - i0 < in_grp ? nin - i0 : in_grp;
         std::vector<int> jobs;
@@ -251,38 +319,48 @@
         if (jobs.empty()) continue;
         const u64 *bin = in + (size_t)i0 * ctw;
         RowMap rm1; rm1.rpg = nl; rm1.gstride_in = ctw; rm1.gstride_out = (size_t)nl * N;
-        SFG_TRY(launch_ntt_inv_map(ctx, bin + (size_t)nl * N, c2, (size_t)ni * nl, pin, rm1));
-        if (pre1) hipLaunchKernelGGL(k_ksw_extend<true>, dim3(N / 512, kc.beta, ni), dim3(256), 0, ctx->stream, c2, ext, kcd, ctx->modc, ctx->tw_fwd);
-        else hipLaunchKernelGGL(k_ksw_extend<false>, dim3(N / 512, kc.beta, ni), dim3(256), 0, ctx->stream, c2, ext, kcd, ctx->modc, ctx->tw_fwd);
+        if (KSW_INV_SPLIT) SFG_TRY(launch_ntt_inv_split(ctx, bin + (size_t)nl * N, c2, (size_t)ni * nl, pin, rm1));
+        else SFG_TRY(launch_ntt_inv_map(ctx, bin + (size_t)nl * N, c2, (size_t)ni * nl, pin, rm1));
+        if (pre1) hipLaunchKernelGGL((k_ksw_extend<true, KSW_INV_SPLIT>), dim3(N / 512, kc.beta, ni), dim3(256), 0, ctx->stream, c2, ext, kcd, ctx->modc, ctx->tw_fwd, ctx->tw_inv);
+        else hipLaunchKernelGGL((k_ksw_extend<false, KSW_INV_SPLIT>), dim3(N / 512, kc.beta, ni), dim3(256), 0, ctx->stream, c2, ext, kcd, ctx->modc, ctx->tw_fwd, ctx->tw_inv);
         SFG_HIP(ctx, hipGetLastError());
         SFG_TRY(launch_ntt_fwd_staged(ctx, ext, extT, (size_t)ni * kc.beta * kc.nt, pext, pre1));
+        std::vector<size_t> tile_at;
         {
             const size_t nj = jobs.size();
             std::vector<const u64 *> kp(nj); std::vector<const uint16_t *> ip(nj); std::vector<u64 *> op(nj); std::vector<int> ii(nj);
             for (size_t k = 0; k < nj; k++) { int jb = jobs[k]; kp[k] = keyp[jb]; ip[k] = idxp[jb]; op[k] = sum ? nullptr : outp[jb]; ii[k] = job_in[jb] - i0; }
+            std::vector<KswTile> tiles, tl;
+            for (size_t c0 = 0; c0 < nj; c0 += chunk) {
+                ksw_job_tiles(kp.data() + c0, ip.data() + c0, (int)(nj - c0 < (size_t)chunk ? nj - c0 : (size_t)chunk), KSW_T, tl);
+                tile_at.push_back(tiles.size()); tiles.insert(tiles.end(), tl.begin(), tl.end());
+            }
+            tile_at.push_back(tiles.size());
             SFG_TRY(sfg_upload_small(ctx, keys_all, kp.data(), nj * sizeof(void *)));
             SFG_TRY(sfg_upload_small(ctx, idx_all, ip.data(), nj * sizeof(void *)));
             if (!sum) SFG_TRY(sfg_upload_small(ctx, out_all, op.data(), nj * sizeof(void *)));
             SFG_TRY(sfg_upload_small(ctx, inidx_all, ii.data(), nj * sizeof(int)));
-        }
-        for (size_t c0 = 0; c0 < jobs.size(); c0 += chunk) {
+            SFG_TRY(sfg_upload_small(ctx, tiles_all, tiles.data(), tiles.size() * sizeof(KswTile)));
+        }
+        for (size_t c0 = 0, ci = 0; c0 < jobs.size(); c0 += chunk, ci++) {
             const int nb = (int)(jobs.size() - c0 < (size_t)chunk ? jobs.size() - c0 : (size_t)chunk);
             const u64 **keys_d = keys_all + c0; const uint16_t **idx_d = idx_all + c0; u64 **out_d = out_all + c0; int *inidx_d = inidx_all + c0;
-            hipLaunchKernelGGL(k_ksw_inner, dim3(N / 512, nq_out + kc.np, nb), dim3(256), 0, ctx->stream, extT, bin, keys_d, inidx_d, acc, kcd, ctx->modc, ctx->nmod, nq_out);
+            const KswTile *tiles_d = tiles_all + tile_at[ci]; const unsigned ntiles = (unsigned)(tile_at[ci + 1] - tile_at[ci]);
+            hipLaunchKernelGGL(k_ksw_inner_p<KSW_T>, dim3(N / 512, kc.np, ntiles), dim3(256), 0, ctx->stream, extT, keys_d, inidx_d, tiles_d, acc, kcd, ctx->modc, ctx->nmod);
             SFG_HIP(ctx, hipGetLastError());
-            RowMap rm4; rm4.rpg = kc.np; rm4.gstride_in = (size_t)kc.nt * N; rm4.gstride_out = (size_t)kc.nt * N;
-            SFG_TRY(launch_ntt_inv_map(ctx, acc + (size_t)nl * N, acc + (size_t)nl * N, (size_t)nb * 2 * kc.np, pp, rm4));
-            if (pre1) hipLaunchKernelGGL(k_moddown_extend<true>, dim3(N / 512, 2, nb), dim3(256), 0, ctx->stream, acc, ext2, kcd, ctx->modc, ctx->tw_fwd, nq_out);
-            else hipLaunchKernelGGL(k_moddown_extend<false>, dim3(N / 512, 2, nb), dim3(256), 0, ctx->stream, acc, ext2, kcd, ctx->modc, ctx->tw_fwd, nq_out);
+            if (KSW_INV_SPLIT) SFG_TRY(launch_ntt_inv_split(ctx, acc, acc, (size_t)nb * 2 * kc.np, pp, rm_dense));
+            else SFG_TRY(launch_ntt_inv(ctx, acc, acc, (size_t)nb * 2 * kc.np, pp));
+            if (pre1) hipLaunchKernelGGL((k_moddown_extend<true, KSW_INV_SPLIT>), dim3(N / 512, 2, nb), dim3(256), 0, ctx->stream, acc, ext2, kcd, ctx->modc, ctx->tw_fwd, ctx->tw_inv, nq_out);
+            else hipLaunchKernelGGL((k_moddown_extend<false, KSW_INV_SPLIT>), dim3(N / 512, 2, nb), dim3(256), 0, ctx->stream, acc, ext2, kcd, ctx->modc, ctx->tw_fwd, ctx->tw_inv, nq_out);
             SFG_HIP(ctx, hipGetLastError());
             SFG_TRY(launch_ntt_fwd_staged(ctx, ext2, ext2T, (size_t)nb * 2 * nl, pq, pre1));
-            if (sum) { SFG_TRY(finish_sum(jobs, c0, nb, bin, inidx_d, idx_d)); continue; }
-            hipLaunchKernelGGL(k_ksw_finish, dim3(N / 256, nq_out, nb), dim3(256), 0, ctx->stream, bin, inidx_d, acc, ext2T, idx_d, out_d, kcd, ctx->modc,
-                               add1 ? add1 + (size_t)i0 * nl * N : nullptr, ff);
+            if (sum) { SFG_TRY(finish_sum(jobs, c0, nb, bin, keys_d, inidx_d, idx_d)); continue; }
+            hipLaunchKernelGGL(k_ksw_finish<KSW_T>, dim3(N / 256, nq_out, ntiles), dim3(256), 0, ctx->stream, extT, bin, keys_d, inidx_d, ext2T, idx_d, out_d, tiles_d, kcd,
+                               ctx->modc, ctx->nmod, add1 ? add1 + (size_t)i0 * nl * N : nullptr, ff);
             SFG_HIP(ctx, hipGetLastError());
         }
     }
-    if (sum) SFG_TRY(finish_sum(std::vector<int>(), 0, 0, in, inidx_all, idx_all));
+    if (sum) SFG_TRY(finish_sum(std::vector<int>(), 0, 0, in, keys_all, inidx_all, idx_all));
     return 0;
 }
 int launch_rotate_right_indexed(sfg_ctx *ctx, const u64 *in, int nin, u64 *out, int nct, int level, const int *nrot_host, const int *in_index) {
```
